# atsuki-ichikawa/KoeMorph

Measured on AMD Instinct MI355X. Metric: blendshape frames/sec (52-coef, 256-win, d_model=256), higher is better.
Workload: dtype f32; 1 GPU; C2: 256 windows/GPU x 136448 samples (8.5 s @16 kHz) -> 1024-pt STFT, hop 533, 80-bin log-mel (257 frames) -> dual-stream attention d_model=256, 8 heads, window 256 -> 52 coefficients + EMA; from audio resident in HBM (rotating batches); windows_per_gpu=256, samples_per_window=136448, parallelism=window-sharded x1, no collective

## Files before the change

include/koemorph.h:

```cpp
#ifndef KOEMORPH_H
#define KOEMORPH_H

#include <stdint.h>

#ifdef __cplusplus
extern "C" {
#endif

#define KM_ABI_VERSION 2

typedef enum km_status {
    KM_OK = 0,
    KM_ERR_INVALID_ARG = -1,
    KM_ERR_UNSUPPORTED = -2,
    KM_ERR_NOT_FINALIZED = -3,
    KM_ERR_WORKSPACE = -4,
    KM_ERR_HIP = -5,
    KM_ERR_NOT_READY = -6
} km_status;

typedef struct km_context* km_handle;

typedef enum km_mel_scale { KM_MEL_SLANEY = 0, KM_MEL_HTK = 1 } km_mel_scale;
typedef enum km_pad_mode { KM_PAD_CONSTANT = 0, KM_PAD_REFLECT = 1 } km_pad_mode;
// ... 121 lines not shown
    float ds_velocity_weight, ds_separation_weight;
    const float* ds_prev_pred_dev;
} km_loss_config;
int km_train_set_loss(km_handle h, const km_loss_config* cfg);
int km_audio_energy(const float* features_dev, int64_t B, int64_t T, int64_t D, float* energy_dev, void* stream);

int km_train_set_dropout(km_handle h, float p, uint64_t seed, int32_t external_masks);
int km_train_get_dropout_step(km_handle h, int64_t* step);
int km_train_set_dropout_step(km_handle h, int64_t step);

int km_train_grad_split(km_handle h, int64_t* early_floats);
int km_train_wait_early(km_handle h, void* stream);
int km_train_get_dropout_masks(km_handle h, int64_t B, uint8_t* mel_host, uint8_t* emo_host, uint8_t* dec_host, void* stream);
int km_train_set_dropout_masks(km_handle h, int64_t B, const uint8_t* mel_host, const uint8_t* emo_host, const uint8_t* dec_host,
                               void* stream);

typedef struct km_legacy_config {
    int32_t abi_version;
    int32_t d_model;
    int32_t num_heads;
    int32_t decoder_hidden;
    int32_t num_blendshapes;
    km_mel_config mel;
} km_legacy_config;
int km_legacy_create(const km_legacy_config* cfg, km_handle* out);
int km_legacy_forward(km_handle h, const float* audio_dev, int64_t B, int64_t L, float* out_dev, void* stream);
int km_legacy_forward_mel(km_handle h, const float* mel_dev, int64_t B, int64_t T_mel, float* out_dev, void* stream);

int km_legacy_train_init(km_handle h, int64_t max_windows, int64_t max_frames, void* stream);
int64_t km_legacy_train_num_params(km_handle h);
int64_t km_legacy_train_param_offset(km_handle h, const char* key);
int km_legacy_train_step_mel(km_handle h, const float* mel_dev, int64_t B, int64_t T, const float* target_dev, float mse_weight,
                             float l1_weight, float* flat_grad_dev, float* loss_dev, float* out_dev, void* stream);
int km_legacy_train_step_audio(km_handle h, const float* audio_dev, int64_t B, int64_t L, const float* target_dev, float mse_weight,
                               float l1_weight, float* flat_grad_dev, float* loss_dev, float* out_dev, void* stream);
int km_legacy_train_set_loss(km_handle h, const km_loss_config* cfg);
int km_legacy_train_adamw(km_handle h, const float* flat_grad_dev, float lr, float beta1, float beta2, float eps,
                          float weight_decay, float max_grad_norm, int64_t step, void* stream);
int km_legacy_train_get_params(km_handle h, float* flat_host, int64_t n);
int km_legacy_train_set_params(km_handle h, const float* flat_host, int64_t n);
int km_legacy_train_get_optimizer_state(km_handle h, float* exp_avg_host, float* exp_avg_sq_host, int64_t n, int32_t* steps2_host);
int km_legacy_train_set_optimizer_state(km_handle h, const float* exp_avg_host, const float* exp_avg_sq_host, int64_t n,
                                        const int32_t* steps2_host);
int km_legacy_train_sync(km_handle h, void* stream);
int km_legacy_train_set_dropout(km_handle h, float p, uint64_t seed, int32_t external_masks);
int km_legacy_train_get_dropout_step(km_handle h, int64_t* step);
int km_legacy_train_set_dropout_step(km_handle h, int64_t step);
int km_legacy_train_get_dropout_masks(km_handle h, int64_t B, int64_t T, uint8_t* enc1_host, uint8_t* enc2_host, uint8_t* attn_host,
                                      uint8_t* dec1_host, uint8_t* dec2_host, void* stream);
int km_legacy_train_set_dropout_masks(km_handle h, int64_t B, int64_t T, const uint8_t* enc1_host, const uint8_t* enc2_host,
                                      const uint8_t* attn_host, const uint8_t* dec1_host, const uint8_t* dec2_host, void* stream);

typedef struct km_koemorph_config {
    int32_t abi_version;
    int32_t mel_dim;
    int32_t emotion_dim;
    int32_t d_model;
    int32_t num_heads;
    int32_t num_encoder_layers;
    int32_t num_attention_layers;
    int32_t decoder_hidden_dim;
    int32_t decoder_layers;
    int32_t decoder_activation;
    int32_t causal;
    int32_t window_size;
    int32_t use_temporal_smoothing;
    int32_t use_constraints;
    int32_t num_blendshapes;
    int32_t output_activation;
    int32_t smoothing_method;
    int32_t smoothing_window;
} km_koemorph_config;
int km_koemorph_create(const km_koemorph_config* cfg, km_handle* out);
int km_koemorph_reserve(km_handle h, int64_t max_batch, int64_t max_frames);
int km_koemorph_forward(km_handle h, const float* mel_dev, const float* emotion_dev, int64_t B, int64_t T,
                        const uint8_t* audio_mask_dev, const float* prev_dev, float* smoother_state_dev,
                        int32_t apply_constraints, float* out_dev, float* raw_dev, float* attn_dev, void* stream);

int km_stream_create(km_handle h, int64_t n_streams, double context_window_s, double update_interval_s,
                     const km_mel_config* mel_cfg);
int km_stream_push(km_handle h, const float* samples_dev, int64_t n_per_stream, void* stream);
int km_stream_tick(km_handle h, const float* emotion_dev, float* out_dev, uint8_t* ready_dev, void* stream);
int km_stream_reset(km_handle h, void* stream);

int km_legacy_stream_create(km_handle h, int64_t n_streams, int64_t buffer_samples, int64_t audio_length);
int km_legacy_stream_push(km_handle h, const float* samples_dev, int64_t n_per_stream, const int32_t* counts_dev, void* stream);
int km_legacy_stream_tick(km_handle h, float* out_dev, uint8_t* ready_dev, void* stream);
int km_legacy_stream_reset(km_handle h, void* stream);

int km_enable_stage_timing(km_handle h, int32_t enable);
int km_stage_times(km_handle h, float* ms3);

int km_egemaps_plan_create(void** plan_out);
int km_egemaps_plan_destroy(void* plan);
int64_t km_egemaps_num_frames(int64_t L);
int64_t km_egemaps_workspace_floats(int64_t B, int64_t L);
int km_egemaps_functionals(void* plan, const float* audio_dev, int64_t B, int64_t L, int32_t normalize, float* work_dev,
                           int64_t work_floats, float* out_dev, void* stream);
int km_egemaps_records(const float* work_dev, int64_t B, int64_t L, float* rec_host, void* stream);
int km_egemaps_track_from_records(float* rec_dev, int64_t B, int64_t nf, void* stream);
int km_egemaps_functionals_from_records(const float* rec_dev, int64_t B, int64_t nf, float* out_dev, void* stream);
int km_linear(const float* x_dev, const float* w_dev, const float* b_dev, int64_t B, int64_t K, int64_t N, float* out_dev, void* stream);

#define KM_METRICS_COUNT 22
int km_metrics_create(void** acc_out);
int km_metrics_destroy(void* acc);
int km_metrics_reset(void* acc, void* stream);
int km_metrics_update(void* acc, const float* pred_dev, const float* target_dev, const float* audio_energy_dev, int64_t N, void* stream);
int km_metrics_compute(void* acc, float* out_dev, void* stream);

enum {
    KM_LOSS_TERM_MSE = 0, KM_LOSS_TERM_L1 = 1, KM_LOSS_TERM_PERCEPTUAL = 2, KM_LOSS_TERM_TEMPORAL = 3, KM_LOSS_TERM_VELOCITY = 4,
    KM_LOSS_TERM_SPARSITY = 5, KM_LOSS_TERM_SMOOTHNESS = 6, KM_LOSS_TERM_LANDMARK = 7, KM_LOSS_TERM_DS_VELOCITY = 8,
    KM_LOSS_TERM_DS_SEPARATION = 9, KM_LOSS_TERM_TOTAL = 10
};
#define KM_LOSS_TERMS 11
int km_loss_terms_create(void** acc_out);
int km_loss_terms_destroy(void* acc);
int km_loss_terms_reset(void* acc, void* stream);
int km_loss_terms_update(void* acc, const km_loss_config* cfg, float mse_weight, float l1_weight,
                         const float* pred_dev, const float* target_dev, int64_t N, float* terms_dev, void* stream);
int km_loss_terms_compute(void* acc, float* out_dev, void* stream);

int km_set_option(km_handle h, const char* name, int64_t value);

int km_debug_buffer(km_handle h, const char* name, float* out, int64_t* n);

int km_resample_labels(const float* src_dev, int64_t n_src, int32_t dims, int64_t n_dst, float* dst_dev, void* stream);
int km_gather_windows(const float* clip_dev, int64_t clip_len, const int32_t* start_frames_dev, int64_t B, int32_t hop,
                      int64_t window_samples, float* audio_out_dev, const float* labels_dev, int64_t n_label_frames,
                      int32_t window_frames, int32_t dims, float* labels_out_dev, float* target_out_dev, void* stream);

int64_t km_format_frames(const float* frames_host, int64_t n_frames, int32_t n_values, const double* timestamps,
                         int32_t newline, char* out, int64_t capacity, int64_t* offsets);

#ifdef __cplusplus
}
#endif
#endif
```

koemorph_amd/_lib.py:

```python
from __future__ import annotations

import ctypes as C
import os
from typing import Optional

from . import build as _build

KM_ABI_VERSION = 2


class KoeMorphError(RuntimeError):
    def __init__(self, code: int, msg: str):
        super().__init__(f"libkoemorph_hip: {msg} (status {code})")
        self.code = code


class KMMelConfig(C.Structure):
    _fields_ = [("sample_rate", C.c_int32), ("n_fft", C.c_int32), ("hop_length", C.c_int32),
                ("n_mels", C.c_int32), ("f_min", C.c_float), ("f_max", C.c_float),
                ("mel_scale", C.c_int32), ("slaney_norm", C.c_int32), ("pad_mode", C.c_int32),
                ("window_norm", C.c_int32), ("log_mode", C.c_int32), ("amin", C.c_float),
                ("top_db", C.c_float), ("db_add", C.c_float), ("db_scale", C.c_float),
                ("log_eps", C.c_float)]

# ... 47 lines not shown
_i64 = C.c_int64
_i32 = C.c_int32
_h = C.c_void_p

SIGNATURES = {
    "km_abi_version": (C.c_int, []),
    "km_last_error": (C.c_char_p, []),
    "km_create": (C.c_int, [C.POINTER(KMConfig), C.POINTER(_h)]),
    "km_destroy": (C.c_int, [_h]),
    "km_load_param": (C.c_int, [_h, C.c_char_p, _p, C.POINTER(_i64), _i32]),
    "km_get_param": (C.c_int, [_h, C.c_char_p, _p, _i64]),
    "km_param_count": (C.c_int, [_h, C.POINTER(_i32), C.POINTER(_i32)]),
    "km_finalize": (C.c_int, [_h, _p]),
    "km_finalize_host": (C.c_int, [_h]),
    "km_reserve": (C.c_int, [_h, _i64, _i64]),
    "km_mel_batch": (C.c_int, [_h, _p, _i64, _i64, _p, _p, _p]),
    "km_mel_num_frames": (_i64, [_h, _i64]),
    "km_mel_extract": (C.c_int, [_h, C.POINTER(KMMelConfig), _p, _i64, _i64, _i64, _p, _p]),
    "km_core_forward": (C.c_int, [_h, _p, _i64, _i64, _p, _p, _p, _p, _p, _p]),
    "km_emotion_logit": (C.c_int, [_h, _p, _i64, _p, _p]),
    "km_core_forward_z": (C.c_int, [_h, _p, _i64, _i64, _p, _p, _p, _p, _p, _p]),
    "km_smooth": (C.c_int, [_h, _p, _p, _i64, _i32, _p]),
    "km_forward_audio": (C.c_int, [_h, _p, _i64, _i64, _p, _p, _p, _i32, _p]),
    "km_forward_clip_supported": (C.c_int, [_h]),
    "km_forward_clip": (C.c_int, [_h, _p, _i64, _p, _i64, _i32, _i32, _p, _p, _p, _i32, _p]),
    "km_forward_audio_pipelined": (C.c_int, [_h, _p, _i64, _i64, _p, _p, _p, _i32, _p]),
    "km_pipeline_flush": (C.c_int, [_h, _p]),
    "km_sequence_num_outputs": (_i64, [_h, _i64, _i32]),
    "km_sequence_forward": (C.c_int, [_h, _p, _i64, _i64, _p, _i32, _i32, _p, _p]),
    "km_ema_scan": (C.c_int, [_h, _p, _i64, _i64, _p]),
    "km_train_init": (C.c_int, [_h, _i64, _p]),
    "km_train_num_params": (_i64, [_h]),
    "km_train_param_offset": (_i64, [_h, C.c_char_p]),
    "km_train_step": (C.c_int, [_h, _p, _i64, _i64, _p, _p, _p, C.c_float, C.c_float, _p, _p, _p, _p, _i32, _p]),
    "km_train_step_audio": (C.c_int, [_h, _p, _i64, _i64, _p, _p, C.c_float, C.c_float, _p, _p, _p, _p, _i32, _p]),
    "km_train_clip_supported": (C.c_int, [_h]),
    "km_train_step_clip": (C.c_int, [_h, _p, _i64, _p, _i64, _i32, _i32, _p, _p, C.c_float, C.c_float, _p, _p, _p, _p, _i32, _p]),
    "km_train_adamw": (C.c_int, [_h, _p, C.c_float, C.c_float, C.c_float, C.c_float, C.c_float, C.c_float, _i64, _p]),
    "km_train_get_params": (C.c_int, [_h, _p, _i64]),
    "km_train_set_params": (C.c_int, [_h, _p, _i64]),
    "km_train_sync": (C.c_int, [_h, _p]),
    "km_train_set_loss": (C.c_int, [_h, C.POINTER(KMLossConfig)]),
    "km_audio_energy": (C.c_int, [_p, _i64, _i64, _i64, _p, _p]),
    "km_train_set_dropout": (C.c_int, [_h, C.c_float, C.c_uint64, _i32]),
    "km_train_get_dropout_step": (C.c_int, [_h, C.POINTER(_i64)]),
    "km_train_set_dropout_step": (C.c_int, [_h, _i64]),
    "km_train_grad_split": (C.c_int, [_h, C.POINTER(_i64)]),
    "km_train_wait_early": (C.c_int, [_h, _p]),
    "km_train_get_dropout_masks": (C.c_int, [_h, _i64, _p, _p, _p, _p]),
    "km_train_set_dropout_masks": (C.c_int, [_h, _i64, _p, _p, _p, _p]),
    "km_train_get_optimizer_state": (C.c_int, [_h, _p, _p, _i64, _p]),
    "km_train_set_optimizer_state": (C.c_int, [_h, _p, _p, _i64, _p]),
    "km_resample_labels": (C.c_int, [_p, C.c_int64, C.c_int32, C.c_int64, _p, _p]),
    "km_gather_windows": (C.c_int, [_p, C.c_int64, _p, C.c_int64, C.c_int32, C.c_int64, _p, _p, C.c_int64, C.c_int32,
                                    C.c_int32, _p, _p, _p]),
    "km_format_frames": (C.c_int64, [_p, C.c_int64, C.c_int32, _p, C.c_int32, _p, C.c_int64, _p]),
    "km_legacy_create": (C.c_int, [C.POINTER(KMLegacyConfig), C.POINTER(_h)]),
    "km_legacy_forward": (C.c_int, [_h, _p, _i64, _i64, _p, _p]),
    "km_legacy_forward_mel": (C.c_int, [_h, _p, _i64, _i64, _p, _p]),
    "km_legacy_train_init": (C.c_int, [_h, _i64, _i64, _p]),
    "km_legacy_train_num_params": (_i64, [_h]),
    "km_legacy_train_param_offset": (_i64, [_h, C.c_char_p]),
    "km_legacy_train_step_mel": (C.c_int, [_h, _p, _i64, _i64, _p, C.c_float, C.c_float, _p, _p, _p, _p]),
    "km_legacy_train_step_audio": (C.c_int, [_h, _p, _i64, _i64, _p, C.c_float, C.c_float, _p, _p, _p, _p]),
    "km_legacy_train_set_loss": (C.c_int, [_h, C.POINTER(KMLossConfig)]),
    "km_legacy_train_adamw": (C.c_int, [_h, _p, C.c_float, C.c_float, C.c_float, C.c_float, C.c_float, C.c_float, _i64, _p]),
    "km_legacy_train_get_params": (C.c_int, [_h, _p, _i64]),
    "km_legacy_train_set_params": (C.c_int, [_h, _p, _i64]),
    "km_legacy_train_get_optimizer_state": (C.c_int, [_h, _p, _p, _i64, _p]),
    "km_legacy_train_set_optimizer_state": (C.c_int, [_h, _p, _p, _i64, _p]),
    "km_legacy_train_sync": (C.c_int, [_h, _p]),
    "km_legacy_train_set_dropout": (C.c_int, [_h, C.c_float, C.c_uint64, _i32]),
    "km_legacy_train_get_dropout_step": (C.c_int, [_h, C.POINTER(_i64)]),
    "km_legacy_train_set_dropout_step": (C.c_int, [_h, _i64]),
    "km_legacy_train_get_dropout_masks": (C.c_int, [_h, _i64, _i64, _p, _p, _p, _p, _p, _p]),
    "km_legacy_train_set_dropout_masks": (C.c_int, [_h, _i64, _i64, _p, _p, _p, _p, _p, _p]),
    "km_koemorph_create": (C.c_int, [C.POINTER(KMKoeMorphConfig), C.POINTER(_h)]),
    "km_koemorph_reserve": (C.c_int, [_h, _i64, _i64]),
    "km_koemorph_forward": (C.c_int, [_h, _p, _p, _i64, _i64, _p, _p, _p, _i32, _p, _p, _p, _p]),
    "km_stream_create": (C.c_int, [_h, _i64, C.c_double, C.c_double, C.POINTER(KMMelConfig)]),
    "km_stream_push": (C.c_int, [_h, _p, _i64, _p]),
    "km_stream_tick": (C.c_int, [_h, _p, _p, _p, _p]),
    "km_stream_reset": (C.c_int, [_h, _p]),
    "km_legacy_stream_create": (C.c_int, [_h, _i64, _i64, _i64]),
    "km_legacy_stream_push": (C.c_int, [_h, _p, _i64, _p, _p]),
    "km_legacy_stream_tick": (C.c_int, [_h, _p, _p, _p]),
    "km_legacy_stream_reset": (C.c_int, [_h, _p]),
    "km_set_option": (C.c_int, [_h, C.c_char_p, _i64]),
    "km_egemaps_plan_create": (C.c_int, [C.POINTER(_p)]),
    "km_egemaps_plan_destroy": (C.c_int, [_p]),
    "km_egemaps_num_frames": (_i64, [_i64]),
    "km_egemaps_workspace_floats": (_i64, [_i64, _i64]),
    "km_egemaps_functionals": (C.c_int, [_p, _p, _i64, _i64, _i32, _p, _i64, _p, _p]),
    "km_egemaps_records": (C.c_int, [_p, _i64, _i64, _p, _p]),
    "km_egemaps_track_from_records": (C.c_int, [_p, _i64, _i64, _p]),
    "km_egemaps_functionals_from_records": (C.c_int, [_p, _i64, _i64, _p, _p]),
    "km_metrics_create": (C.c_int, [C.POINTER(_p)]),
    "km_metrics_destroy": (C.c_int, [_p]),
    "km_metrics_reset": (C.c_int, [_p, _p]),
    "km_metrics_update": (C.c_int, [_p, _p, _p, _p, _i64, _p]),
    "km_metrics_compute": (C.c_int, [_p, _p, _p]),
    "km_loss_terms_create": (C.c_int, [C.POINTER(_p)]),
    "km_loss_terms_destroy": (C.c_int, [_p]),
    "km_loss_terms_reset": (C.c_int, [_p, _p]),
    "km_loss_terms_update": (C.c_int, [_p, C.POINTER(KMLossConfig), C.c_float, C.c_float, _p, _p, _i64, _p, _p]),
    "km_loss_terms_compute": (C.c_int, [_p, _p, _p]),
    "km_linear": (C.c_int, [_p, _p, _p, _i64, _i64, _i64, _p, _p]),
    "km_enable_stage_timing": (C.c_int, [_h, _i32]),
    "km_stage_times": (C.c_int, [_h, C.POINTER(C.c_float)]),
    "km_debug_buffer": (C.c_int, [_h, C.c_char_p, _p, C.POINTER(_i64)]),
}

_lib: Optional[C.CDLL] = None


def load(build_if_missing: bool = True) -> C.CDLL:
    global _lib
    if _lib is not None:
        return _lib
    path = _build.LIB_PATH
    if os.environ.get("KM_LIBRARY"):
        path, build_if_missing = os.environ["KM_LIBRARY"], False
    if build_if_missing and _build.is_stale():
        try:
            _build.build_library()
        except Exception as exc:
            if not os.path.exists(path) or os.environ.get("KM_ALLOW_STALE") != "1":
                raise KoeMorphError(KM_ERR_HIP, f"libkoemorph_hip.so is missing or older than its sources and the rebuild "
                                                f"failed ({exc}); set KM_ALLOW_STALE=1 to load the stale library") from exc
            import warnings
            warnings.warn(f"libkoemorph_hip.so is OLDER than its sources and the rebuild failed ({exc}); "
                          "loading the stale library (KM_ALLOW_STALE=1)", RuntimeWarning, stacklevel=2)
    if not os.path.exists(path):
        raise KoeMorphError(KM_ERR_HIP, f"{path} is missing: run `python -m koemorph_amd.build` "
                                        "(there is no CPU fallback)")
    import torch
    lib = C.CDLL(path)
    for name, (res, args) in SIGNATURES.items():
        fn = getattr(lib, name)
        fn.restype = res
        fn.argtypes = args
    if lib.km_abi_version() != KM_ABI_VERSION:
        raise KoeMorphError(KM_ERR_INVALID_ARG, "ABI version mismatch between _lib.py and the shared library")
    _lib = lib
    return lib


def check(code: int) -> None:
    if code != KM_OK:
        msg = load().km_last_error()
        raise KoeMorphError(code, msg.decode("utf-8", "replace") if msg else "unknown error")
```

koemorph_amd/csrc/km_api.hip:

```cpp
#include <hip/hip_runtime.h>

#include <cstdlib>

#include <cstring>
#include <vector>

#include "km_context.h"
#include "km_device.h"
#include "km_gemm.h"

using namespace km;

#define HIP_TRY(expr)                                                                         \
    do {                                                                                      \
        hipError_t e_ = (expr);                                                               \
        if (e_ != hipSuccess) {                                                                                                        \
            (void)hipGetLastError();  \
            return fail(KM_ERR_HIP, "%s: %s", #expr, hipGetErrorString(e_));                                                           \
        }                                                                                                                              \
    } while (0)

static int free_streams(Context* c);
static int free_train(Context* c);
static int free_pipeline(Context* c);
// ... 702 lines not shown
    c->kmm_batch = Bm; c->kmm_frames = Tm;
    return KM_OK;
}

int km_koemorph_forward(km_handle h, const float* mel_dev, const float* emotion_dev, int64_t B, int64_t T,
                        const uint8_t* audio_mask_dev, const float* prev_dev, float* smoother_state_dev,
                        int32_t apply_constraints, float* out_dev, float* raw_dev, float* attn_dev, void* stream) {
    if (int rc = need_ready(h)) return rc;
    Context* c = h;
    if (c->kind != 2) return fail(KM_ERR_INVALID_ARG, "not a KoeMorphModel handle (km_koemorph_create)");
    if (!mel_dev || !emotion_dev || !out_dev || B <= 0 || T <= 0) return fail(KM_ERR_INVALID_ARG, "km_koemorph_forward: bad argument");
    if (!c->ws_generic || B * koemorph_ws_floats(c, T) > c->kmm_batch * koemorph_ws_floats(c, c->kmm_frames))
        return fail(KM_ERR_WORKSPACE, "workspace too small for %lld x %lld frames: call km_koemorph_reserve", (long long)B, (long long)T);
    return launch_koemorph(c, mel_dev, emotion_dev, B, T, audio_mask_dev, prev_dev, smoother_state_dev, apply_constraints, out_dev, raw_dev,
                           attn_dev, stream);
}

int km_legacy_forward(km_handle h, const float* audio_dev, int64_t B, int64_t L, float* out_dev, void* stream) {
    if (int rc = need_ready(h)) return rc;
    Context* c = h;
    if (c->kind != 1) return fail(KM_ERR_INVALID_ARG, "not a legacy handle (km_legacy_create)");
    if (!audio_dev || !out_dev || B <= 0 || L <= 0) return fail(KM_ERR_INVALID_ARG, "km_legacy_forward: bad argument");
    const int64_t n_frames = 1 + L / c->cfg.mel.hop_length;
    if (B > c->ws_windows || n_frames > c->ws_frames || !c->ws_generic)
        return fail(KM_ERR_WORKSPACE, "workspace too small for %lld windows x %lld samples: call km_reserve",
                    (long long)B, (long long)L);
    if (legacy_pow_ok(c)) {
        if (int rc = launch_mel_power(c, c->mel_plans[0], mel_windows(audio_dev, B, L), stream)) return rc;
        const LogParams lp = plan_log_params(c->mel_plans[0]);
        const LegacyPowSrc src{c->ws_melpow, c->ws_melmax, &lp};
        return launch_legacy(c, nullptr, B, n_frames, out_dev, stream, &src);
    }
    if (int rc = launch_mel(c, c->mel_plans[0], mel_windows(audio_dev, B, L), 0, c->ws_mel, nullptr, stream)) return rc;
    return launch_legacy(c, c->ws_mel, B, n_frames, out_dev, stream);
}

int km_ema_scan(km_handle h, float* x_dev, int64_t B, int64_t N, void* stream) {
    if (int rc = need_ready(h)) return rc;
    if (h->kind != 0) return fail(KM_ERR_INVALID_ARG, "this entry point needs a dual-stream handle (km_create)");
    if (!x_dev || B <= 0 || N <= 0) return fail(KM_ERR_INVALID_ARG, "km_ema_scan: bad argument");
    return launch_ema_scan(h, x_dev, B, N, stream);
}

int km_smooth(km_handle h, float* x_dev, float* state_dev, int64_t B, int32_t first, void* stream) {
    if (int rc = need_ready(h)) return rc;
    if (!x_dev || !state_dev || B <= 0) return fail(KM_ERR_INVALID_ARG, "km_smooth: bad argument");
    return launch_smooth(h, x_dev, state_dev, B, first, stream);
}

int km_forward_audio(km_handle h, const float* audio_dev, int64_t B, int64_t L, const float* emotion_dev,
                     float* out_dev, float* state_dev, int32_t first, void* stream) {
    if (int rc = need_dual(h)) return rc;
    Context* c = h;
    if (!audio_dev || !emotion_dev || !out_dev || B <= 0 || L <= 0)
        return fail(KM_ERR_INVALID_ARG, "km_forward_audio: bad argument");
    const int64_t n_frames = 1 + L / c->cfg.mel.hop_length;
    if (B > c->ws_windows || n_frames > c->ws_frames)
        return fail(KM_ERR_WORKSPACE, "workspace too small for %lld windows x %lld samples: call km_reserve",
                    (long long)B, (long long)L);
    MelPlan* plan = c->mel_plans[0];
    const MelSrc src = mel_windows(audio_dev, B, L);
    if (!c->fused_ok) {
        if (!c->ws_generic) return fail(KM_ERR_WORKSPACE, "generic workspace missing: call km_reserve after km_finalize");
        const bool power_path = generic_core_takes_power(c) && !c->opt.generic_staged;
        const bool fuse_emo = power_path && mel_fuses_emotion(c, plan);
        if (!fuse_emo)
            if (int rc = launch_emotion(c, emotion_dev, B, c->ws_zemo, stream)) return rc;
        if (power_path) {
            if (int rc = launch_mel_power(c, plan, src, stream, fuse_emo ? mel_emotion(emotion_dev, c->ws_zemo) : MelCarry{})) return rc;
            if (int rc = launch_core_generic_power(c, plan, B, n_frames, c->ws_zemo, out_dev, nullptr, nullptr, stream)) return rc;
        } else if (c->NK == 80 && !c->opt.generic_staged) {
            float* xp = generic_packed_x(c, B);
            if (int rc = launch_mel_packed(c, plan, src, xp, c->T, (c->KT + 15) / 16 * 16, stream)) return rc;
            if (int rc = launch_core_generic_packed(c, xp, B, c->ws_zemo, out_dev, nullptr, nullptr, stream)) return rc;
        } else {
            if (int rc = launch_mel(c, plan, src, 0, c->ws_mel, c->ws_short, stream)) return rc;
            if (int rc = launch_core_generic(c, c->ws_mel, B, n_frames, c->ws_short, c->ws_zemo, out_dev, nullptr, nullptr, stream)) return rc;
        }
        if (state_dev) return launch_smooth(c, out_dev, state_dev, B, first, stream);
        return KM_OK;
    }
    hipStream_t st = (hipStream_t)stream;
    const bool tm = c->stage_timing;
    const bool fuse_emo = mel_fuses_emotion(c, plan);
    if (tm) HIP_TRY(hipEventRecord((hipEvent_t)c->stage_ev[0], st));
    if (!fuse_emo)
        if (int rc = launch_emotion(c, emotion_dev, B, c->ws_zemo, stream)) return rc;
    if (tm) HIP_TRY(hipEventRecord((hipEvent_t)c->stage_ev[1], st));
    if (int rc = launch_mel_power(c, plan, src, stream, fuse_emo ? mel_emotion(emotion_dev, c->ws_zemo) : MelCarry{})) return rc;
    if (tm) { HIP_TRY(hipEventRecord((hipEvent_t)c->stage_ev[2], st)); HIP_TRY(hipEventRecord((hipEvent_t)c->stage_ev[3], st)); }
    if (int rc = launch_core_fused_db(c, plan, B, n_frames, c->ws_zemo, out_dev, stream, core_workspace(state_dev, first))) return rc;
    if (tm) HIP_TRY(hipEventRecord((hipEvent_t)c->stage_ev[4], st));
    return KM_OK;
}

static bool forward_clip_ok(Context* c) {
    if (c->mel_plans.empty() || !c->fused_ok || c->opt.core_split == 3 || c->opt.core_split == 6) return false;
    return mel_rp_ok(c, c->mel_plans[0]) && clip_frames_shared(c, c->mel_plans[0]);
}

int km_forward_clip_supported(km_handle h) {
    if (!h || !h->dev_finalized || h->kind != 0) return 0;
    return forward_clip_ok(h) ? 1 : 0;
}

int km_forward_clip(km_handle h, const float* clip_dev, int64_t clip_len, const int32_t* start_frames_dev, int64_t B,
                    int32_t min_start_frame, int32_t max_start_frame, const float* emotion_dev, float* out_dev,
                    float* state_dev, int32_t first, void* stream) {
    if (int rc = need_dual(h)) return rc;
    Context* c = h;
    if (!clip_dev || !start_frames_dev || !emotion_dev || !out_dev || B <= 0 || clip_len <= 0 || min_start_frame < 0 ||
        max_start_frame < min_start_frame)
        return fail(KM_ERR_INVALID_ARG, "km_forward_clip: bad argument");
    const km_mel_config& m = c->mel_plans[0]->cfg;
    if (!forward_clip_ok(c))
        return fail(KM_ERR_UNSUPPORTED, "km_forward_clip: needs the fused core (d_model 256, window 256, 8 heads) behind the 1024-point "
                    "front end with constant padding and hop >= n_fft / 2 (hop %d, n_fft %d): gather the windows (km_gather_windows) "
                    "and call km_forward_audio", m.hop_length, m.n_fft);
    const int64_t T = c->T, hop = m.hop_length;
    const int64_t n_span = (int64_t)(max_start_frame - min_start_frame) + T + 1;
    if (clip_len >= (1ll << 31) || ((int64_t)max_start_frame + T + 2) * hop >= (1ll << 31) || n_span * c->NK >= (1ll << 31))
        return fail(KM_ERR_INVALID_ARG, "km_forward_clip: clip or start frame beyond 2^31 samples");
    if (B > c->ws_windows)
        return fail(KM_ERR_WORKSPACE, "workspace holds %lld windows, need %lld: call km_reserve", (long long)c->ws_windows, (long long)B);
    if (int rc = grow_buffer(&c->fwd_span, &c->fwd_span_cap, n_span, c->NK * sizeof(float), stream, "km_forward_clip: span frames")) return rc;
    if (int rc = grow_buffer(&c->fwd_edge, &c->fwd_edge_cap, B, 2 * c->NK * sizeof(float), stream, "km_forward_clip: windows")) return rc;
    if (int rc = launch_emotion(c, emotion_dev, B, c->ws_zemo, stream)) return rc;
    if (int rc = launch_mel_clip_span(c, c->mel_plans[0], clip_dev, clip_len, start_frames_dev, B, min_start_frame, n_span, (int)T,
                                      c->fwd_span, c->fwd_edge, stream)) return rc;
    if (int rc = launch_clip_window_max(c, c->fwd_span, c->fwd_edge, start_frames_dev, B, min_start_frame, n_span, (int)(T + 1),
                                        stream)) return rc;
    const ClipTable tab{c->fwd_span, c->fwd_edge, (int)n_span, start_frames_dev, min_start_frame};
    return launch_core_fused_db(c, c->mel_plans[0], B, T + 1, c->ws_zemo, out_dev, stream, core_table(&tab, state_dev, first));
}

static int free_streams(Context* c) {
    void* ptrs[] = {c->ring, c->ring_wptr, c->ring_frames, c->ring_ready, c->ring_started, c->ring_state};
    for (void* p : ptrs)
        if (p) HIP_TRY(hipFree(p));
    c->ring = nullptr; c->ring_wptr = nullptr; c->ring_frames = nullptr; c->ring_ready = nullptr;
    c->ring_started = nullptr; c->ring_state = nullptr; c->n_streams = 0;
    return KM_OK;
}

int km_stream_reset(km_handle h, void* stream) {
    if (int rc = need_dual(h)) return rc;
    Context* c = h;
    if (c->n_streams <= 0) return fail(KM_ERR_INVALID_ARG, "km_stream_reset: no streams (km_stream_create first)");
    hipStream_t st = (hipStream_t)stream;
    HIP_TRY(hipMemsetAsync(c->ring, 0, (size_t)c->n_streams * c->ring_len * sizeof(float), st));
    HIP_TRY(hipMemsetAsync(c->ring_wptr, 0, (size_t)c->n_streams * sizeof(int), st));
    HIP_TRY(hipMemsetAsync(c->ring_frames, 0, (size_t)c->n_streams * sizeof(int), st));
    HIP_TRY(hipMemsetAsync(c->ring_ready, 0, (size_t)c->n_streams, st));
    HIP_TRY(hipMemsetAsync(c->ring_started, 0, (size_t)c->n_streams, st));
    HIP_TRY(hipMemsetAsync(c->ring_state, 0, (size_t)c->n_streams * c->NB * sizeof(float), st));
    return KM_OK;
}

int km_stream_create(km_handle h, int64_t n_streams, double context_window_s, double update_interval_s,
                     const km_mel_config* mel_cfg) {
    if (int rc = need_dual(h)) return rc;
    Context* c = h;
    if (n_streams <= 0 || !(context_window_s > 0) || !(update_interval_s > 0) || !mel_cfg)
        return fail(KM_ERR_INVALID_ARG, "km_stream_create: bad argument");
    if (mel_cfg->n_fft != 512 && mel_cfg->n_fft != 1024) return fail(KM_ERR_UNSUPPORTED, "n_fft must be 512 or 1024");
    if (mel_cfg->n_mels != c->NK) return fail(KM_ERR_INVALID_ARG, "stream front end must produce %d mel channels", c->NK);
    if (int rc = free_streams(c)) return rc;
    const int sr = mel_cfg->sample_rate;
    c->ring_len = (int64_t)(context_window_s * sr);
    const double target_fps = 1.0 / update_interval_s;
    c->ring_hop = (int)((double)sr / target_fps);
    c->stream_out_frames = (int64_t)(context_window_s / update_interval_s);
    if (c->ring_hop <= 0 || c->ring_len <= mel_cfg->n_fft / 2) return fail(KM_ERR_INVALID_ARG, "context window too short");
    c->n_streams = n_streams;
    HIP_TRY(hipMalloc(reinterpret_cast<void**>(&c->ring), (size_t)n_streams * c->ring_len * sizeof(float)));
    HIP_TRY(hipMalloc(reinterpret_cast<void**>(&c->ring_wptr), (size_t)n_streams * sizeof(int)));
    HIP_TRY(hipMalloc(reinterpret_cast<void**>(&c->ring_frames), (size_t)n_streams * sizeof(int)));
    HIP_TRY(hipMalloc(reinterpret_cast<void**>(&c->ring_ready), (size_t)n_streams));
    HIP_TRY(hipMalloc(reinterpret_cast<void**>(&c->ring_started), (size_t)n_streams));
    HIP_TRY(hipMalloc(reinterpret_cast<void**>(&c->ring_state), (size_t)n_streams * c->NB * sizeof(float)));
    c->stream_plan = find_or_add_plan(c, *mel_cfg);
    if (int rc = upload_mel_plan(c->stream_plan)) return rc;
    if (int rc = km_reserve(h, n_streams, c->ring_len)) return rc;
    if (int rc = km_stream_reset(h, nullptr)) return rc;
    HIP_TRY(hipDeviceSynchronize());
    return KM_OK;
}

int km_stream_push(km_handle h, const float* samples_dev, int64_t n_per_stream, void* stream) {
    if (int rc = need_dual(h)) return rc;
    Context* c = h;
    if (c->n_streams <= 0) return fail(KM_ERR_INVALID_ARG, "km_stream_push: no streams (km_stream_create first)");
    if (!samples_dev) return fail(KM_ERR_INVALID_ARG, "km_stream_push: NULL samples");
    const int64_t diff = n_per_stream - c->ring_hop;
    if (diff > 1 || diff < -1)
        return fail(KM_ERR_INVALID_ARG, "Frame size mismatch: expected ~%d, got %lld", c->ring_hop, (long long)n_per_stream);
    return launch_ring_push(c, samples_dev, n_per_stream, stream);
}

int km_stream_tick(km_handle h, const float* emotion_dev, float* out_dev, uint8_t* ready_dev, void* stream) {
    if (int rc = need_dual(h)) return rc;
    Context* c = h;
    if (c->n_streams <= 0) return fail(KM_ERR_INVALID_ARG, "km_stream_tick: no streams (km_stream_create first)");
    if (!emotion_dev || !out_dev) return fail(KM_ERR_INVALID_ARG, "km_stream_tick: NULL argument");
    if (!c->fused_ok && !core512_stream_ok(c))
        return fail(KM_ERR_UNSUPPORTED, "no kernel for d_model=%d, mel_sequence_length=%d, heads=%d", c->d, c->T, c->H);
    const int64_t S = c->n_streams, L = c->ring_len;
    const int64_t n_frames = 1 + L / c->stream_plan->cfg.hop_length;
    if (S > c->ws_windows || n_frames > c->ws_frames) return fail(KM_ERR_WORKSPACE, "stream workspace too small");
    const bool fuse_emo = mel_fuses_emotion(c, c->stream_plan);
    if (!fuse_emo)
        if (int rc = launch_emotion(c, emotion_dev, S, c->ws_zemo, stream)) return rc;
    if (int rc = launch_mel_power(c, c->stream_plan, mel_rings(c), stream, fuse_emo ? mel_emotion(emotion_dev, c->ws_zemo) : MelCarry{})) return rc;
    if (c->fused_ok) {
        if (int rc = launch_core_fused_db(c, c->stream_plan, S, n_frames, c->ws_zemo, out_dev, stream, core_stream(c))) return rc;
    } else {
        if (int rc = launch_core512_stream(c, c->stream_plan, S, n_frames, c->ws_zemo, out_dev, stream)) return rc;
    }
    if (ready_dev)
        HIP_TRY(hipMemcpyAsync(ready_dev, c->ring_ready, (size_t)S, hipMemcpyDeviceToDevice, (hipStream_t)stream));
    return KM_OK;
}

static int free_legacy_streams(Context* c) {
    void* ptrs[] = {c->lfifo, c->lfifo_state, c->lfifo_stage, c->lfifo_ready, c->lfifo_attn};
    for (void* p : ptrs)
        if (p) HIP_TRY(hipFree(p));
    c->lfifo = nullptr; c->lfifo_state = nullptr; c->lfifo_stage = nullptr; c->lfifo_ready = nullptr; c->lfifo_attn = nullptr;
    c->lfifo_cap = c->lfifo_state_cap = c->lfifo_stage_cap = c->lfifo_ready_cap = c->lfifo_attn_cap = 0;
    c->lfifo_streams = c->lfifo_len = c->lfifo_window = 0;
    return KM_OK;
}

static bool legacy_stream_ok(Context* c) {
    return c->legacy_fused && c->legacy_tail_fused && c->d == 256 && c->H == 8 && c->legacy_hidden == 128 && c->NB == 52 && c->NK == 80 &&
           !c->mel_plans.empty() && c->mel_plans[0]->cfg.n_fft == 1024 && legacy_pow_ok(c);
}

static int need_legacy_stream(Context* c, const char* who) {
    if (int rc = need_ready(c)) return rc;
    if (c->kind != 1) return fail(KM_ERR_INVALID_ARG, "%s needs a legacy handle (km_legacy_create)", who);
    if (c->lfifo_streams <= 0) return fail(KM_ERR_INVALID_ARG, "%s: no streams (km_legacy_stream_create first)", who);
    return KM_OK;
}

int km_legacy_stream_reset(km_handle h, void* stream) {
    if (int rc = need_legacy_stream(h, "km_legacy_stream_reset")) return rc;
    Context* c = h;
    hipStream_t st = (hipStream_t)stream;
    const size_t S = (size_t)c->lfifo_streams;
    HIP_TRY(hipMemsetAsync(c->lfifo, 0, S * c->lfifo_len * sizeof(float), st));
    HIP_TRY(hipMemsetAsync(c->lfifo_stage, 0, S * c->lfifo_window * sizeof(float), st));
    HIP_TRY(hipMemsetAsync(c->lfifo_state, 0, 3 * S * sizeof(int), st));
    HIP_TRY(hipMemsetAsync(c->lfifo_ready, 0, S, st));
    return KM_OK;
}

int km_legacy_stream_create(km_handle h, int64_t n_streams, int64_t buffer_samples, int64_t audio_length) {
    if (int rc = need_ready(h)) return rc;
    Context* c = h;
    if (c->kind != 1) return fail(KM_ERR_INVALID_ARG, "km_legacy_stream_create needs a legacy handle (km_legacy_create)");
    if (n_streams <= 0 || buffer_samples <= 0 || audio_length <= 0 || audio_length > buffer_samples || n_streams >= (1ll << 24) ||
        buffer_samples >= (1ll << 30))
        return fail(KM_ERR_INVALID_ARG, "km_legacy_stream_create: bad argument (%lld streams, buffer of %lld samples, windows of %lld)",
                    (long long)n_streams, (long long)buffer_samples, (long long)audio_length);
    const int64_t T = 1 + audio_length / c->cfg.mel.hop_length;
    if (!legacy_stream_ok(c))
        return fail(KM_ERR_UNSUPPORTED, "km_legacy_stream_create: windows of %lld frames are served for d_model 256, 8 heads, decoder hidden 128 "
                    "behind the 1024-point front end only (got d_model %d, %d heads, hidden %d, n_fft %d)", (long long)T, c->d, c->H,
                    c->legacy_hidden, c->mel_plans.empty() ? 0 : c->mel_plans[0]->cfg.n_fft);
    if (T > 32)
        return fail(KM_ERR_UNSUPPORTED, "km_legacy_stream_create: windows of %lld samples are %lld frames, the stream kernel holds at most 32 "
                    "(use km_legacy_forward for longer windows)", (long long)audio_length, (long long)T);
    c->lfifo_streams = 0;
    const char* what = "km_legacy_stream_create";
    if (int rc = grow_buffer(&c->lfifo, &c->lfifo_cap, n_streams * buffer_samples, sizeof(float), nullptr, what)) return rc;
    if (int rc = grow_buffer(&c->lfifo_state, &c->lfifo_state_cap, 3 * n_streams, sizeof(int), nullptr, what)) return rc;
    if (int rc = grow_buffer(&c->lfifo_stage, &c->lfifo_stage_cap, n_streams * audio_length, sizeof(float), nullptr, what)) return rc;
    if (int rc = grow_buffer(&c->lfifo_ready, &c->lfifo_ready_cap, n_streams, 1, nullptr, what)) return rc;
    if (int rc = grow_buffer(&c->lfifo_attn, &c->lfifo_attn_cap, n_streams * c->NB * c->d, sizeof(float), nullptr, what)) return rc;
    if (int rc = km_reserve(h, n_streams, audio_length)) return rc;
    if (!legacy_stream_ok(c)) return fail(KM_ERR_UNSUPPORTED, "km_legacy_stream_create: the power-mel workspace is not 16-byte aligned");
    c->lfifo_streams = n_streams; c->lfifo_len = buffer_samples; c->lfifo_window = audio_length;
    HIP_TRY(hipMemset(c->ws_melmax, 0, (size_t)c->ws_windows * sizeof(unsigned)));
    c->melmax_dirty = false;
    if (int rc = km_legacy_stream_reset(h, nullptr)) return rc;
    if (int rc = km_legacy_stream_tick(h, c->lfifo_attn, nullptr, nullptr)) return rc;
    HIP_TRY(hipDeviceSynchronize());
    return KM_OK;
}

int km_legacy_stream_push(km_handle h, const float* samples_dev, int64_t n_per_stream, const int32_t* counts_dev, void* stream) {
    if (int rc = need_legacy_stream(h, "km_legacy_stream_push")) return rc;
    if (!samples_dev || n_per_stream <= 0 || n_per_stream >= (1ll << 30))
        return fail(KM_ERR_INVALID_ARG, "km_legacy_stream_push: bad argument");
    return launch_lfifo_push(h, samples_dev, n_per_stream, counts_dev, stream);
}

// ... 12 lines not shown

int km_enable_stage_timing(km_handle h, int32_t enable) {
    if (!h) return fail(KM_ERR_INVALID_ARG, "NULL handle");
    Context* c = h;
    if (enable && !c->stage_ev[0])
        for (int i = 0; i < 5; ++i) {
            hipEvent_t e;
            HIP_TRY(hipEventCreate(&e));
            c->stage_ev[i] = e;
        }
    c->stage_timing = enable != 0;
    return KM_OK;
}

int km_stage_times(km_handle h, float* ms3) {
    if (!h || !ms3) return fail(KM_ERR_INVALID_ARG, "km_stage_times: NULL argument");
    Context* c = h;
    if (!c->stage_ev[0]) return fail(KM_ERR_INVALID_ARG, "stage timing was never enabled");
    HIP_TRY(hipEventSynchronize((hipEvent_t)c->stage_ev[4]));
    HIP_TRY(hipEventElapsedTime(&ms3[0], (hipEvent_t)c->stage_ev[0], (hipEvent_t)c->stage_ev[1]));
    HIP_TRY(hipEventElapsedTime(&ms3[1], (hipEvent_t)c->stage_ev[1], (hipEvent_t)c->stage_ev[2]));
    HIP_TRY(hipEventElapsedTime(&ms3[2], (hipEvent_t)c->stage_ev[3], (hipEvent_t)c->stage_ev[4]));
    return KM_OK;
}

static int free_pipeline(Context* c) {
    for (int i = 0; i < 2; ++i) {
        if (c->pipe_melpow[i]) HIP_TRY(hipFree(c->pipe_melpow[i]));
        if (c->pipe_melmax[i]) HIP_TRY(hipFree(c->pipe_melmax[i]));
        if (c->pipe_zemo[i]) HIP_TRY(hipFree(c->pipe_zemo[i]));
        c->pipe_melpow[i] = nullptr; c->pipe_melmax[i] = nullptr; c->pipe_zemo[i] = nullptr; c->pipe_dirty[i] = true;
    }
    c->pipe_windows = c->pipe_frames = 0;
    return KM_OK;
}

static int ensure_pipeline(Context* c, int64_t B, int64_t n_frames) {
    if (!c->pipe_s1) {
        hipStream_t s;
        HIP_TRY(hipStreamCreateWithFlags(&s, hipStreamNonBlocking)); c->pipe_s1 = s;
        HIP_TRY(hipStreamCreateWithFlags(&s, hipStreamNonBlocking)); c->pipe_s2 = s;
        for (int i = 0; i < 2; ++i) {
            hipEvent_t e;
            HIP_TRY(hipEventCreateWithFlags(&e, hipEventDisableTiming)); c->pipe_ev_in[i] = e;
            HIP_TRY(hipEventCreateWithFlags(&e, hipEventDisableTiming)); c->pipe_ev_mel[i] = e;
            HIP_TRY(hipEventCreateWithFlags(&e, hipEventDisableTiming)); c->pipe_ev_core[i] = e;
        }
    }
    if (B <= c->pipe_windows && n_frames <= c->pipe_frames) return KM_OK;
    HIP_TRY(hipDeviceSynchronize());
    if (int rc = free_pipeline(c)) return rc;
    const int64_t W = B, F = n_frames;
    for (int i = 0; i < 2; ++i) {
        HIP_TRY(hipMalloc(reinterpret_cast<void**>(&c->pipe_melpow[i]), (size_t)W * F * c->NK * sizeof(float)));
        HIP_TRY(hipMalloc(reinterpret_cast<void**>(&c->pipe_melmax[i]), (size_t)W * sizeof(unsigned)));
        HIP_TRY(hipMalloc(reinterpret_cast<void**>(&c->pipe_zemo[i]), (size_t)W * sizeof(float)));
    }
    c->pipe_windows = W; c->pipe_frames = F; c->pipe_seq = 0;
    return KM_OK;
}

int km_forward_audio_pipelined(km_handle h, const float* audio_dev, int64_t B, int64_t L, const float* emotion_dev,
                               float* out_dev, float* state_dev, int32_t first, void* stream) {
    if (int rc = need_dual(h)) return rc;
    Context* c = h;
    if (!audio_dev || !emotion_dev || !out_dev || B <= 0 || L <= 0)
        return fail(KM_ERR_INVALID_ARG, "km_forward_audio_pipelined: bad argument");
    if (!c->fused_ok) return fail(KM_ERR_UNSUPPORTED, "the pipelined mode needs the fused kernel shape (d_model 256, window 256, 8 heads)");
    const int64_t n_frames = 1 + L / c->cfg.mel.hop_length;
    if (B > c->ws_windows || n_frames > c->ws_frames)
        return fail(KM_ERR_WORKSPACE, "workspace too small for %lld windows x %lld samples: call km_reserve", (long long)B, (long long)L);
    if (int rc = ensure_pipeline(c, B > c->ws_windows ? B : c->ws_windows, n_frames > c->ws_frames ? n_frames : c->ws_frames)) return rc;
    const int slot = (int)(c->pipe_seq & 1);
    hipStream_t caller = (hipStream_t)stream, s1 = (hipStream_t)c->pipe_s1, s2 = (hipStream_t)c->pipe_s2;
    const bool tm = c->stage_timing;
    float* keep_pow = c->ws_melpow; unsigned* keep_max = c->ws_melmax; float* keep_z = c->ws_zemo; const bool keep_dirty = c->melmax_dirty;
    c->ws_melpow = c->pipe_melpow[slot]; c->ws_melmax = c->pipe_melmax[slot]; c->ws_zemo = c->pipe_zemo[slot];
    c->melmax_dirty = c->pipe_dirty[slot];
    int rc = KM_OK;
    do {
        if (hipEventRecord((hipEvent_t)c->pipe_ev_in[slot], caller) != hipSuccess) { rc = fail(KM_ERR_HIP, "hipEventRecord failed"); break; }
        if (hipStreamWaitEvent(s1, (hipEvent_t)c->pipe_ev_in[slot], 0) != hipSuccess) { rc = fail(KM_ERR_HIP, "hipStreamWaitEvent failed"); break; }
        if (tm) (void)hipEventRecord((hipEvent_t)c->stage_ev[0], s1);
        const bool fuse_emo = mel_fuses_emotion(c, c->mel_plans[0]);
        if (!fuse_emo && (rc = launch_emotion(c, emotion_dev, B, c->ws_zemo, s1))) break;
        if (tm) (void)hipEventRecord((hipEvent_t)c->stage_ev[1], s1);
        if ((rc = launch_mel_power(c, c->mel_plans[0], mel_windows(audio_dev, B, L), s1, fuse_emo ? mel_emotion(emotion_dev, c->ws_zemo) : MelCarry{}))) break;
        if (tm) (void)hipEventRecord((hipEvent_t)c->stage_ev[2], s1);
        (void)hipEventRecord((hipEvent_t)c->pipe_ev_mel[slot], s1);
        (void)hipStreamWaitEvent(s2, (hipEvent_t)c->pipe_ev_mel[slot], 0);
        if (tm) (void)hipEventRecord((hipEvent_t)c->stage_ev[3], s2);
        if ((rc = launch_core_fused_db(c, c->mel_plans[0], B, n_frames, c->ws_zemo, out_dev, s2, core_workspace(state_dev, first)))) break;
        if (tm) (void)hipEventRecord((hipEvent_t)c->stage_ev[4], s2);
        (void)hipEventRecord((hipEvent_t)c->pipe_ev_core[slot], s2);
        if (c->pipe_seq > 0) (void)hipStreamWaitEvent(caller, (hipEvent_t)c->pipe_ev_core[slot ^ 1], 0);
    } while (0);
    c->pipe_dirty[slot] = c->melmax_dirty;
    c->ws_melpow = keep_pow; c->ws_melmax = keep_max; c->ws_zemo = keep_z; c->melmax_dirty = keep_dirty;
    if (rc == KM_OK) c->pipe_seq += 1;
    return rc;
}

int km_pipeline_flush(km_handle h, void* stream) {
    if (int rc = need_dual(h)) return rc;
    Context* c = h;
    if (c->pipe_seq > 0 && c->pipe_s1)
        HIP_TRY(hipStreamWaitEvent((hipStream_t)stream, (hipEvent_t)c->pipe_ev_core[(c->pipe_seq - 1) & 1], 0));
    return KM_OK;
}

int64_t km_sequence_num_outputs(km_handle h, int64_t L, int32_t stride_frames) {
    if (!h || L < 0 || stride_frames <= 0) return -1;
    const int64_t num_frames = L / h->cfg.mel.hop_length;
    const int64_t n = (num_frames - h->T) / stride_frames + 1;
    const int64_t nn = (num_frames - h->T) >= 0 ? n : ((num_frames - h->T - (stride_frames - 1)) / stride_frames + 1);
    return nn > 1 ? nn : 1;
}

int km_sequence_forward(km_handle h, const float* audio_dev, int64_t B, int64_t L, const float* emotion_dev,
                        int32_t stride_frames, int32_t smooth, float* out_dev, void* stream) {
    if (int rc = need_dual(h)) return rc;
    Context* c = h;
    if (!audio_dev || !emotion_dev || !out_dev || B <= 0 || L <= 0 || stride_frames <= 0)
        return fail(KM_ERR_INVALID_ARG, "km_sequence_forward: bad argument");
    if (!c->fused_ok && !c->ws_generic)
        return fail(KM_ERR_WORKSPACE, "generic workspace missing: call km_reserve after km_finalize");
    const int hop = c->cfg.mel.hop_length;
    const int64_t N = km_sequence_num_outputs(h, L, stride_frames);
    const int64_t W = (int64_t)c->T * hop;
    const int64_t step = (int64_t)stride_frames * hop;
    const int64_t n_frames = 1 + W / hop;
    if (c->ws_windows < B || c->ws_windows < 1 || n_frames > c->ws_frames)
        return fail(KM_ERR_WORKSPACE, "workspace too small for %lld clips / %lld-frame windows: call km_reserve",
                    (long long)B, (long long)n_frames);
    if (N > 0x7fffffff) return fail(KM_ERR_INVALID_ARG, "too many output frames");
    const int64_t total = B * N, tile = c->ws_windows;
    const bool dedup = !c->opt.seq_per_window;
    MelPlan* plan = c->mel_plans[0];
    const bool shared = c->fused_ok && dedup && mel_rp_ok(c, plan) && N < (1 << 24);
    const int64_t nfc = (N - 1) * stride_frames + n_frames;
    if (shared) {
        const char* what = "km_sequence_forward: clip frames / windows";
        if (int rc = grow_buffer(&c->seq_pow, &c->seq_pow_cap, B * nfc, c->NK * sizeof(float), stream, what)) return rc;
        if (int rc = grow_buffer(&c->seq_fmax, &c->seq_fmax_cap, B * nfc, sizeof(unsigned), stream, what)) return rc;
        if (int rc = grow_buffer(&c->seq_edge, &c->seq_edge_cap, total, 2 * c->NK * sizeof(float), stream, what)) return rc;
        if (int rc = grow_buffer(&c->seq_emax, &c->seq_emax_cap, total, 2 * sizeof(unsigned), stream, what)) return rc;
    }
    if (int rc = launch_emotion(c, emotion_dev, B, c->ws_zemo, stream)) return rc;
    if (shared) {
        hipStream_t st = (hipStream_t)stream;
        HIP_TRY(hipMemsetAsync(c->seq_fmax, 0, (size_t)B * nfc * sizeof(unsigned), st));
        HIP_TRY(hipMemsetAsync(c->seq_emax, 0, (size_t)total * 2 * sizeof(unsigned), st));
        const SeqFrames clip_img{c->seq_pow, c->seq_fmax, nfc, 1};
        if (int rc = launch_mel_power(c, plan, mel_clip_windows(audio_dev, L, B, (nfc - 1) * hop, 0, 0, 1), stream, mel_to_frames(&clip_img))) return rc;
        const SeqFrames edge_img{c->seq_edge, c->seq_emax, 2, (int)(n_frames - 1)};
        if (int rc = launch_mel_power(c, plan, mel_clip_windows(audio_dev, L, total, W, step, 0, (int)N), stream, mel_to_frames(&edge_img))) return rc;
        const SeqCore sc{c->seq_pow, c->seq_edge, (int)nfc, (int)stride_frames, (int)N};
        for (int64_t w0 = 0; w0 < total; w0 += tile) {
            const int64_t nw = (total - w0) < tile ? (total - w0) : tile;
            if (int rc = launch_seq_window_max(c, c->seq_fmax, c->seq_emax, nw, w0, (int)nfc, (int)stride_frames, (int)N,
                                               (int)n_frames, stream)) return rc;
            if (int rc = launch_core_fused_db(c, plan, nw, n_frames, c->ws_zemo, out_dev + w0 * c->NB, stream, core_strided(&sc, w0))) return rc;
        }
        if (smooth) return launch_ema_scan(c, out_dev, B, N, stream);
        return KM_OK;
    }
    for (int64_t w0 = 0; w0 < total; w0 += tile) {
        const int64_t nw = (total - w0) < tile ? (total - w0) : tile;
        const MelSrc src = mel_clip_windows(audio_dev, L, nw, W, step, w0, (int)N);
        if (c->fused_ok) {
            if (int rc = launch_mel_power(c, plan, src, stream)) return rc;
            if (int rc = launch_core_fused_db(c, plan, nw, n_frames, c->ws_zemo, out_dev + w0 * c->NB, stream, core_workspace_seq(w0, (int)N))) return rc;
        } else {
            if (int rc = launch_mel(c, plan, src, 0, c->ws_mel, c->ws_short, stream)) return rc;
            if (int rc = launch_gather_clip_logits(c, c->ws_zemo, c->ws_zemo_win, nw, w0, (int)N, stream)) return rc;
// ... 10 lines not shown
```

koemorph_amd/csrc/km_context.h:

```cpp
#pragma once

#include <cstdint>
#include <map>
#include <string>
#include <vector>

#include "koemorph.h"

namespace km {

constexpr int kNumMouth = 28;
constexpr int kNumExpr = 24;
extern const int kMouthIdx[kNumMouth];
extern const int kExprIdx[kNumExpr];

struct HostParam {
    std::vector<int64_t> shape;
    std::vector<float> data;
    bool loaded = false;
};

struct Packed {
    std::vector<float> host;
    float* dev = nullptr;
};

constexpr int kMelRpWaves = 8;
constexpr int kMelRpGroups = 4;
constexpr int kMelRpRow = 580;

struct MelPlan {
    km_mel_config cfg{};
    int n_freq = 0;
    std::vector<float> window;
    std::vector<float> twiddle;
    std::vector<int32_t> fb_start;
    std::vector<int32_t> fb_count;
    std::vector<int32_t> fb_offset;
    std::vector<float> fb_weight;
    std::vector<int32_t> fbg_gid;
    std::vector<int32_t> fbg_desc;
    std::vector<float> fbg_weight;
    int fbg_extent = 0;
    float* d_window = nullptr;
    float* d_twiddle = nullptr;
    int32_t* d_fb_start = nullptr;
    int32_t* d_fb_count = nullptr;
    int32_t* d_fb_offset = nullptr;
    float* d_fb_weight = nullptr;
    int32_t* d_fbg_gid = nullptr;
    int32_t* d_fbg_desc = nullptr;
    float* d_fbg_weight = nullptr;
    bool uploaded = false;
};

struct Options {
    int core_split = 0;
    int seq_per_window = 0;
    int generic_staged = 0;
    int mel_two_frame = 0;
    int emotion_separate = 0;
    int no_ln_fusion = 0, no_db_fusion = 0, no_score_fusion = 0, no_out_fusion = 0, no_v_fusion = 0;
    int legacy_no_merge = 0;
    int no_core_merge = 0;
    int legacy_no_tail_fusion = 0;
    int legacy_no_enc_fusion = 0;
    int legacy_no_attn_fusion = 0;
    int kmm_no_fuse = 0;
    int train_no_split = 0;
    int train_split_min_k = 0;
    int train_alone_max = 0;
    int train_no_dy_split = 0;
    int train_ln_fuse_rows = 0;
    int train_no_ln_fuse = 0;
    int train_colsum_gemm = 0;
    int train_no_fe_pack = 0;
    int train_attn_regs = 0;
    int train_no_dma = 0;
    int train_op_per_launch = 0;
    int train_bm32_below = 0;
    int train_tail_groups = 0;
};
void options_from_env(Options& o);
int set_option(struct Context* c, const char* name, long long value);

struct PerDeviceOnce {
    unsigned long long seen[4] = {0, 0, 0, 0};
    bool first(int device) {
        if (device < 0 || device >= 256) return true;
        const unsigned long long bit = 1ull << (device & 63);
        if (seen[device >> 6] & bit) return false;
        seen[device >> 6] |= bit;
        return true;
    }
};

struct Context {
    km_config cfg{};
    Options opt{};
    int kind = 0;
    int legacy_hidden = 128;
    km_koemorph_config kmm{};
    int64_t kmm_batch = 0, kmm_frames = 0;
    bool legacy_tail_fused = false;
    bool legacy_fused = false;
    bool kmm_fused = false;
    int d = 0, H = 0, hd = 0, T = 0, KT = 0, ED = 0, DH = 0, NB = 0, NK = 0;
    std::map<std::string, HostParam> params;
    std::vector<std::string> param_order;
    std::map<std::string, Packed> packed;
    bool host_finalized = false;
    bool dev_finalized = false;
    bool fused_ok = false;
    float alpha = 0.0f;
    int device = -1;

    std::vector<MelPlan*> mel_plans;

    int64_t ws_windows = 0, ws_samples = 0;
    float* ws_zemo = nullptr;
    float* ws_zemo_win = nullptr;
    float* ws_melpow = nullptr;
    unsigned* ws_melmax = nullptr;
    unsigned* ws_chunkctr = nullptr;
    int64_t ws_chunkctr_cap = 0;
    float* ws_mel = nullptr;
    float* ws_short = nullptr;
    float* ws_generic = nullptr;
    int64_t ws_frames = 0;
    int ws_mels = 0;
    int64_t n_streams = 0, ring_len = 0;
    int ring_hop = 0;
    float* ring = nullptr;
    int* ring_wptr = nullptr;
    int* ring_frames = nullptr;
    unsigned char* ring_ready = nullptr;
    unsigned char* ring_started = nullptr;
    float* ring_state = nullptr;
    MelPlan* stream_plan = nullptr;
    int64_t stream_out_frames = 0;
    int64_t lfifo_streams = 0, lfifo_len = 0, lfifo_window = 0;
    float* lfifo = nullptr; int64_t lfifo_cap = 0;
    int* lfifo_state = nullptr; int64_t lfifo_state_cap = 0;
    float* lfifo_stage = nullptr; int64_t lfifo_stage_cap = 0;
    unsigned char* lfifo_ready = nullptr; int64_t lfifo_ready_cap = 0;
    float* lfifo_attn = nullptr; int64_t lfifo_attn_cap = 0;
    int64_t tr_nparams = 0, tr_windows = 0;
    int64_t tr_early = 0;
    void* tr_early_ev = nullptr;
    bool tr_early_recorded = false;
    std::map<std::string, int64_t> tr_offset;
    float* tr_params = nullptr; float* tr_m = nullptr; float* tr_v = nullptr;
    float* trp_wcep = nullptr;
    float* tr_part = nullptr; float* tr_gnorm = nullptr; float* tr_loss = nullptr;
    int* tr_steps = nullptr;
    bool tr_alpha_live = false;
    km_loss_config tr_loss_cfg{};
    float* trp_act = nullptr; int64_t trp_act_floats = 0;
    float* trp_split = nullptr; int64_t trp_split_floats = 0;
    float* trp_tail_part = nullptr; unsigned* trp_tail_ctr = nullptr;
    void* trp_masks = nullptr;
    int* trp_drop_ctr = nullptr;
    float tr_dropout_p = 0.f;
    int tr_dropout_mode = 0;
    unsigned long long tr_dropout_seed = 0;
    float* ltr_ws = nullptr; int64_t ltr_ws_floats = 0;
    int64_t ltr_frames = 0;
    float* ltr_part = nullptr;
    unsigned char* ltr_masks = nullptr; int64_t ltr_mask_bytes = 0;
    int64_t ltr_mask_B = 0, ltr_mask_T = 0;
    float* seq_pow = nullptr; unsigned* seq_fmax = nullptr; float* seq_edge = nullptr; unsigned* seq_emax = nullptr;
    int64_t seq_pow_cap = 0, seq_fmax_cap = 0, seq_edge_cap = 0, seq_emax_cap = 0;
    float* fwd_span = nullptr; float* fwd_edge = nullptr;
    int64_t fwd_span_cap = 0, fwd_edge_cap = 0;
    float* clip_span = nullptr; float* clip_edge = nullptr;
    int64_t clip_span_cap = 0, clip_edge_cap = 0;
    int64_t tr_alpha_steps = 0;
    bool stage_timing = false;
    void* stage_ev[6] = {nullptr, nullptr, nullptr, nullptr, nullptr, nullptr};
    void* pipe_s1 = nullptr; void* pipe_s2 = nullptr;
    void* pipe_ev_in[2] = {nullptr, nullptr}; void* pipe_ev_mel[2] = {nullptr, nullptr}; void* pipe_ev_core[2] = {nullptr, nullptr};
    float* pipe_melpow[2] = {nullptr, nullptr}; unsigned* pipe_melmax[2] = {nullptr, nullptr}; float* pipe_zemo[2] = {nullptr, nullptr};
    bool pipe_dirty[2] = {true, true};
    int64_t pipe_seq = 0, pipe_windows = 0, pipe_frames = 0;
    bool melmax_dirty = true;
};

void set_error(const char* fmt, ...);
int fail(int code, const char* fmt, ...);

int finalize_host(Context* c);
MelPlan* build_mel_plan(const km_mel_config& cfg);
MelPlan* find_or_add_plan(Context* c, const km_mel_config& cfg);

int launch_emotion(Context* c, const float* emo, int64_t B, float* zemo, void* stream);
int launch_core_fused(Context* c, const float* mel, int64_t B, int64_t T_in, const float* mel_short,
                      const float* zemo, float* out, float* raw, float* attn, float* state, int first,
                      void* stream);
struct SeqCore {
    const float* pow;
    const float* edge;
    int nfc, stride, n_per_clip;
};
struct ClipTable {
    const float* span;
    const float* edge;
    int n_span;
    const int* start; int min_start;
};
struct CoreSrc {
    float* state; int first;
    int64_t win0; int zemo_div;
    int64_t n_use;
    const unsigned char* ready; unsigned char* started;
    const SeqCore* seq;
    const ClipTable* tab;
};
inline CoreSrc core_workspace(float* state, int first) { return {state, first, 0, 1, 0, nullptr, nullptr, nullptr, nullptr}; }
inline CoreSrc core_workspace_seq(int64_t win0, int n_per_clip) { return {nullptr, 1, win0, n_per_clip, 0, nullptr, nullptr, nullptr, nullptr}; }
inline CoreSrc core_strided(const SeqCore* s, int64_t win0) { return {nullptr, 1, win0, s->n_per_clip, 0, nullptr, nullptr, s, nullptr}; }
inline CoreSrc core_table(const ClipTable* t, float* state, int first) { return {state, first, 0, 1, 0, nullptr, nullptr, nullptr, t}; }
inline CoreSrc core_stream(Context* c) { return {c->ring_state, 0, 0, 1, c->stream_out_frames, c->ring_ready, c->ring_started, nullptr, nullptr}; }
int launch_core_fused_db(Context* c, MelPlan* p, int64_t B, int64_t n_frames, const float* zemo, float* out, void* stream,
                         const CoreSrc& src);
int launch_seq_window_max(Context* c, const unsigned* fmax, const unsigned* emax, int64_t nw, int64_t win0, int nfc, int stride,
                          int n_per_clip, int n_frames, void* stream);
int launch_clip_window_max(Context* c, const float* span, const float* edge, const int* start, int64_t B, int min_start,
                           int64_t n_span, int n_frames, void* stream);
int launch_ema_scan(Context* c, float* x, int64_t B, int64_t N, void* stream);
int launch_smooth(Context* c, float* x, float* state, int64_t B, int first, void* stream);

int train_refresh_padded_weights(Context* c, void* stream);
int train_adamw(Context* c, const float* flat_grad, float lr, float b1, float b2, float eps, float wd, float max_norm,
                int64_t step, void* stream);

int64_t trainp_act_floats(Context* c, int64_t* fixed);
int64_t trainp_kp(Context* c);
int64_t trainp_mask_alloc_bytes(Context* c);
int trainp_mask_sizes(Context* c, int64_t B, int64_t* mel, int64_t* emo, int64_t* dec);
int trainp_copy_masks(Context* c, int64_t B, unsigned char* mel, unsigned char* emo, unsigned char* dec, int to_device, void* stream);
struct LogParams;
struct TrainAudioSrc { const float* melpow; const unsigned* melmax; int n_frames; const LogParams* lp; bool packed; };
struct TrainStepArgs {
    const float* emo; const float* target; float mse_w, l1_w; float* flat_grad; float* loss_dev; float* out_dev;
    float* ema_state; int ema_first; void* stream;
};
int train_forward_backward(Context* c, const float* mel, int64_t B, int64_t T_in, const float* mel_short, const float* xp_dev,
                           const TrainAudioSrc* asrc, const TrainStepArgs& a);
int launch_audio_energy(const float* feats, int64_t B, int64_t T, int64_t D, float* out, void* stream);

bool legacy_train_supported(Context* c);
int legacy_train_init(Context* c, int64_t max_windows, int64_t max_frames, void* stream);
float* legacy_train_mel_buffer(Context* c);
int legacy_train_step(Context* c, const float* mel, int64_t B, int64_t T, const float* target, float mse_w, float l1_w, float* grad,
                      float* loss_dev, float* out_dev, void* stream);
int legacy_train_copy_masks(Context* c, int64_t B, int64_t T, unsigned char* const host[5], int to_device, void* stream);

int64_t generic_ws_floats(Context* c);
int64_t legacy_ws_floats(Context* c, int64_t frames);
int finalize_host_legacy(Context* c);
int finalize_host_koemorph(Context* c);
int64_t koemorph_ws_floats(Context* c, int64_t T);
int launch_koemorph(Context* c, const float* mel, const float* emo, int64_t B, int64_t T, const unsigned char* kvalid, const float* prev,
                    float* state, int apply_constraints, float* out, float* raw, float* attn, void* stream);
struct LegacyPowSrc { const float* melpow; unsigned* melmax; const LogParams* lp; };
bool legacy_pow_ok(Context* c);
int launch_legacy(Context* c, const float* mel, int64_t B, int64_t T_mel, float* out, void* stream, const LegacyPowSrc* pow_src = nullptr);
int launch_gather_clip_logits(Context* c, const float* zclip, float* zwin, int64_t nw, int64_t w0, int wins_per_clip, void* stream);
int launch_core_generic_packed(Context* c, const float* xp, int64_t B, const float* zemo, float* out, float* raw, float* attn,
                               void* stream);
float* generic_packed_x(Context* c, int64_t B);
bool generic_core_takes_power(Context* c);
int launch_core_generic_power(Context* c, MelPlan* plan, int64_t B, int64_t n_frames, const float* zemo, float* out,
                              float* raw, float* attn, void* stream);
int launch_core_generic(Context* c, const float* mel, int64_t B, int64_t T_in, const float* mel_short, const float* zemo,
                        float* out, float* raw, float* attn, void* stream);
bool core512_stream_ok(Context* c);
int launch_core512_stream(Context* c, MelPlan* plan, int64_t S, int64_t n_frames, const float* zemo, float* out, void* stream);

struct SeqFrames {
    float* pow;
    unsigned* fmax;
    int64_t n_rows;
    int frame_mul;
};
struct MelPack { float* xt; int T, KP; };
struct MelSrc {
    const float* audio; int64_t B, L;
    int64_t clip_len, win_step, win0; int wins_per_clip;
    const int* ring_start; const unsigned char* ready;
};
inline MelSrc mel_windows(const float* audio, int64_t B, int64_t L) { return {audio, B, L, L, 0, 0, 1, nullptr, nullptr}; }
inline MelSrc mel_clip_windows(const float* clips, int64_t clip_len, int64_t B, int64_t L, int64_t win_step, int64_t win0, int wins_per_clip) {
    return {clips, B, L, clip_len, win_step, win0, wins_per_clip, nullptr, nullptr};
}
inline MelSrc mel_rings(Context* c) { return {c->ring, c->n_streams, c->ring_len, c->ring_len, 0, 0, 1, c->ring_wptr, c->ring_ready}; }
struct MelCarry { const float* emotion = nullptr; float* zemo = nullptr; const SeqFrames* seq = nullptr; const MelPack* pack = nullptr; };
inline MelCarry mel_emotion(const float* emotion, float* zemo) { return {emotion, zemo, nullptr, nullptr}; }
inline MelCarry mel_to_frames(const SeqFrames* seq) { return {nullptr, nullptr, seq, nullptr}; }
inline MelCarry mel_to_pack(const MelPack* pack) { return {nullptr, nullptr, nullptr, pack}; }
int launch_mel_power(Context* c, MelPlan* p, const MelSrc& src, void* stream, const MelCarry& carry = {});
bool mel_rp_ok(Context* c, MelPlan* p);
bool clip_frames_shared(Context* c, MelPlan* p);
bool mel_packs(Context* c, MelPlan* p, int64_t n_frames, int64_t T);
int launch_mel_clip_span(Context* c, MelPlan* p, const float* clip, int64_t clip_len, const int* start_frames, int64_t B,
                         int min_start, int64_t n_span, int T, float* span, float* edge, void* stream);
int launch_train_clip_pack(Context* c, MelPlan* p, const float* span, const float* edge, const int* start_frames, int64_t B,
                           int min_start, int64_t n_span, int T, int KP, float* xt, void* stream);
bool mel_fuses_emotion(Context* c, MelPlan* p);
int ensure_chunk_counters(Context* c, int64_t windows, void* stream);
int growth_refused(void* stream, const char* what, int64_t need, int64_t cap);
int grow_buffer(void* ptr_addr, int64_t* cap, int64_t need, size_t unit_bytes, void* stream, const char* what);
int launch_ring_push(Context* c, const float* samples, int64_t n_per_stream, void* stream);

int launch_lfifo_push(Context* c, const float* samples, int64_t n_per_stream, const int* counts, void* stream);
int launch_lfifo_pop(Context* c, unsigned char* ready_out, void* stream);
int launch_legacy_stream_model(Context* c, const float* melpow, unsigned* melmax, const unsigned char* ready, int64_t S, int Tm,
                               const LogParams& lp, float* O, float* out, void* stream);
int launch_mel(Context* c, MelPlan* p, const MelSrc& src, int64_t out_frames, float* mel_long, float* mel_short, void* stream);
int launch_mel_packed(Context* c, MelPlan* p, const MelSrc& src, float* xp, int T, int KP, void* stream);
int upload_mel_plan(MelPlan* p);
void free_mel_plan(MelPlan* p);

}

struct km_context : public km::Context {};
```

koemorph_amd/csrc/km_core.hip:

```cpp
#include <hip/hip_runtime.h>

#include <type_traits>

#include "km_context.h"
#include "km_device.h"

namespace km {

typedef float f32x4 __attribute__((ext_vector_type(4)));
#define KM_MFMA(a, b, c) __builtin_amdgcn_mfma_f32_16x16x4f32((a), (b), (c), 0, 0, 0)

#define HIP_TRY(expr)                                                                         \
    do {                                                                                      \
        hipError_t e_ = (expr);                                                               \
        if (e_ != hipSuccess) {                                                                                                        \
            (void)hipGetLastError();  \
            return fail(KM_ERR_HIP, "%s: %s", #expr, hipGetErrorString(e_));                                                           \
        }                                                                                                                              \
    } while (0)

namespace fused {
constexpr int D = 256, T = 256, NK = 80, NQ = 28, DH = 128;
constexpr int KT = 259, KTP = 264, YS = 264, NW = 8, NT = 512;
constexpr int KP = 33;
constexpr int KB = 16;
constexpr int R1_FLOATS = KTP * NK;
constexpr int R2_FLOATS = 2 * NW * NK + 2 * NK;
constexpr int LDS_BYTES = (R1_FLOATS + R2_FLOATS) * 4;
constexpr int YSB = 264;
constexpr int PLANE_FLOATS = NK * YSB / 2;
constexpr int XSB = 296, XKB = 9;
constexpr int XPLANE_FLOATS = NK * XSB / 2;
constexpr int r1_floats(int np) { return np * XPLANE_FLOATS > R1_FLOATS ? np * XPLANE_FLOATS : R1_FLOATS; }
constexpr int lds_bytes(int np) { return (r1_floats(np) + R2_FLOATS) * 4; }
}

typedef __bf16 bf16x8 __attribute__((ext_vector_type(8)));
typedef unsigned int u32x4c __attribute__((ext_vector_type(4)));

struct CoreArgs {
    const float* mel;
    const float* mel_short;
    const float* zemo;
    int t_in;
    const float *wce_p, *bce, *ln_g, *ln_b, *qk_p, *wv_p, *wf_p, *bf, *w2, *b2, *wsum;
    const void* qkv_s;
    const void* wce_s;
    float* out;
    float* raw;
    float* attn;
    float* state;
    int first;
    float alpha;
    const float* melpow;
    unsigned* melmax;
    int n_frames;
    LogParams lp;
    int64_t win0;
    int zemo_div;
    int n_use;
    const float* seq_pow;
    const float* seq_edge;
    int seq_nfc, seq_stride, seq_n;
    const unsigned char* ready;
    unsigned char* started;
    const int* seq_start;
    int seq_min;
};

__device__ __forceinline__ int mouth_slot_of(int i) { return (i >= 14 && i <= 40) ? i - 14 : (i == 51 ? 27 : -1); }

template <bool ATTN, bool FUSE_DB, int NP = 0, bool TAB = false>
__global__ __launch_bounds__(512) void core_fused_kernel(CoreArgs a) {
    using namespace fused;
    extern __shared__ __attribute__((aligned(16))) float smem[];
    float* R1 = smem;
    float* R2 = smem + r1_floats(NP);

    const int b = blockIdx.x;
    const int tid = threadIdx.x;
    const int lane = tid & 63;
    const int wave = __builtin_amdgcn_readfirstlane(tid >> 6);
    const int g = lane >> 4, j = lane & 15;
    if constexpr (FUSE_DB) {
        if (a.ready && !a.ready[b]) return;
    }

    const int n0 = 32 * wave + j;
    float4 bw0 = make_float4(0.f, 0.f, 0.f, 0.f), bw1 = bw0;
    if constexpr (NP == 0) {
        const float4* wp0 = reinterpret_cast<const float4*>(a.wce_p) + (size_t)wave * KP * 64 + lane;
        bw0 = wp0[0];
    }
    const float bb0 = a.bce[n0], bb1 = a.bce[n0 + 16];
    const float g0 = a.ln_g[n0], g1 = a.ln_g[n0 + 16], be0 = a.ln_b[n0], be1 = a.ln_b[n0 + 16];
    float bf4[4], w24[4];
#pragma unroll
    for (int r = 0; r < 4; ++r) { bf4[r] = a.bf[16 * wave + 4 * g + r]; w24[r] = a.w2[16 * wave + 4 * g + r]; }
    const float tail_b2 = a.b2[0], tail_ws = tid < 52 ? a.wsum[tid] : 0.f;

    if constexpr (FUSE_DB) {
        float ref_db, floor_db;
        log_window_consts(a.lp, __uint_as_float(a.melmax[b]), ref_db, floor_db);
        const int F = a.n_frames;
        const int U = a.n_use;
        const int tv = U < T ? U : T;
        const float4* src = reinterpret_cast<const float4*>(a.melpow + (int64_t)b * F * NK);
        const float4 *seq_rows = nullptr, *seq_e = nullptr;
        if constexpr (TAB) {
            int r0 = a.seq_start[b];
            r0 = (r0 < 0 ? 0 : r0) - a.seq_min;
            r0 = r0 < 0 ? 0 : (r0 > a.seq_nfc - F ? a.seq_nfc - F : r0);
            seq_rows = reinterpret_cast<const float4*>(a.seq_pow + (int64_t)r0 * NK);
            seq_e = reinterpret_cast<const float4*>(a.seq_edge + (int64_t)b * 2 * NK);
        } else if (a.seq_pow) {
            const int64_t gw = a.win0 + b, clip = gw / a.seq_n, wi = gw - clip * a.seq_n;
            seq_rows = reinterpret_cast<const float4*>(a.seq_pow + (clip * a.seq_nfc + wi * a.seq_stride) * NK);
            seq_e = reinterpret_cast<const float4*>(a.seq_edge + gw * 2 * NK);
        }
        auto row4 = [&](int fr) -> const float4* {
            if (!seq_rows) return src + fr * 20;
            return fr == 0 ? seq_e : (fr == F - 1 ? seq_e + 20 : seq_rows + fr * 20);
        };
        float4* dst = reinterpret_cast<float4*>(R1);
        const float4 z4 = make_float4(0.f, 0.f, 0.f, 0.f);
        if constexpr (NP > 0) {
            auto src_row = [&](int t) -> int {
                if (t < T) return t < tv ? (t < F ? t : F - 1) : -1;
                if (t >= T + 3) return -1;
                const int r = t - T;
                int fr = -1;
                if (U >= 3) fr = U - 3 + r; else if (r < U) fr = r;
                return fr >= F ? F - 1 : fr;
            };
            auto stage_planes = [&](auto mode) {
                constexpr int MODE = decltype(mode)::value;
#pragma unroll 1
                for (int unit = tid; unit < XKB * 4 * 20; unit += NT) {
                    const int t8 = unit / 20, c4 = unit - t8 * 20;
                    float4 xv8[8];
                    unsigned okm = 0;
#pragma unroll
                    for (int q = 0; q < 8; ++q) {
                        const int fr = src_row(8 * t8 + q);
                        okm |= (fr >= 0 ? 1u : 0u) << q;
                        xv8[q] = fr >= 0 ? row4(fr)[c4] : z4;
                    }
                    float xe[4][8];
#pragma unroll
                    for (int q = 0; q < 8; ++q) {
                        const float4 v = (okm >> q) & 1 ? log_four_t<MODE>(a.lp, xv8[q], ref_db, floor_db) : z4;
                        xe[0][q] = v.x; xe[1][q] = v.y; xe[2][q] = v.z; xe[3][q] = v.w;
                    }
                    unsigned short* xp = reinterpret_cast<unsigned short*>(R1) + (4 * c4) * XSB + 8 * t8;
#pragma unroll
                    for (int pc = 0; pc < NP; ++pc)
#pragma unroll
                        for (int e = 0; e < 4; ++e) {
                            bf16x8 pk;
#pragma unroll
                            for (int q = 0; q < 8; ++q) {
                                const __bf16 pbf = (__bf16)xe[e][q];
                                pk[q] = pbf;
                                xe[e][q] -= (float)pbf;
                            }
                            *reinterpret_cast<bf16x8*>(xp + pc * (NK * XSB) + e * XSB) = pk;
                        }
                }
            };
            if (a.lp.log_mode == KM_LOG_LN_EPS) stage_planes(std::integral_constant<int, KM_LOG_LN_EPS>{});
            else stage_planes(std::integral_constant<int, KM_LOG_DB_MAX>{});
        } else {
        constexpr int NLD = T * 20 / NT;
        static_assert(NLD * NT == T * 20, "phase 0 assumes T*20 is a multiple of the workgroup size");
        float4 xv[NLD];
#pragma unroll
        for (int u = 0; u < NLD; ++u) {
            const int i = tid + NT * u;
            int fr = i / 20;
            const int c4 = i - fr * 20;
            fr = fr < F ? fr : F - 1;
            xv[u] = i < tv * 20 ? row4(fr)[c4] : z4;
        }
        float4 sv = z4;
        bool s_ok = false;
        if (tid < 60) {
            const int r = tid / 20;
            int fr = -1;
            if (U >= 3) fr = U - 3 + r; else if (r < U) fr = r;
            if (fr >= F) fr = F - 1;
            s_ok = fr >= 0;
            if (s_ok) sv = row4(fr)[tid - r * 20];
        }
        auto convert = [&](auto mode) {
            constexpr int MODE = decltype(mode)::value;
#pragma unroll
            for (int u = 0; u < NLD; ++u) {
                const int i = tid + NT * u;
                dst[i] = i < tv * 20 ? log_four_t<MODE>(a.lp, xv[u], ref_db, floor_db) : z4;
            }
            if (tid < 60) dst[T * 20 + tid] = s_ok ? log_four_t<MODE>(a.lp, sv, ref_db, floor_db) : z4;
        };
        if (a.lp.log_mode == KM_LOG_LN_EPS) convert(std::integral_constant<int, KM_LOG_LN_EPS>{});
        else convert(std::integral_constant<int, KM_LOG_DB_MAX>{});
        if (tid >= 64 && tid < 64 + (KTP - KT) * 20) dst[KT * 20 + tid - 64] = z4;
        }
    } else {
        const int tv = a.t_in < T ? a.t_in : T;
        const float4* src = reinterpret_cast<const float4*>(a.mel + (int64_t)b * a.t_in * NK);
        float4* dst = reinterpret_cast<float4*>(R1);
        const float4 z4 = make_float4(0.f, 0.f, 0.f, 0.f);
        for (int i = tid; i < tv * 20; i += NT) dst[i] = src[i];
        for (int i = tv * 20 + tid; i < T * 20; i += NT) dst[i] = z4;
        const float4* s4 = reinterpret_cast<const float4*>(a.mel_short + (int64_t)b * 3 * NK);
        if (tid < 60) dst[T * 20 + tid] = s4[tid];
        if (tid >= 64 && tid < 64 + (KTP - KT) * 20) dst[KT * 20 + tid - 64] = z4;
    }
    __syncthreads();
    if constexpr (FUSE_DB) {
        if (tid == 0) a.melmax[b] = 0u;
    }

    f32x4 acc[5][2];
#pragma unroll
    for (int mt = 0; mt < 5; ++mt) { acc[mt][0] = f32x4{0, 0, 0, 0}; acc[mt][1] = f32x4{0, 0, 0, 0}; }
    if constexpr (NP > 0) {
        const u32x4c* wp = reinterpret_cast<const u32x4c*>(a.wce_s) + (size_t)wave * XKB * 2 * NP * 64 + lane;
        const unsigned short* Xp = reinterpret_cast<const unsigned short*>(R1) + j * XSB + 8 * g;
        u32x4c bw[2][NP];
#pragma unroll
        for (int t = 0; t < 2; ++t)
#pragma unroll
            for (int pc = 0; pc < NP; ++pc) bw[t][pc] = wp[(t * NP + pc) * 64];
        for (int kb = 0; kb < XKB; ++kb) {
            const int kn = kb + 1 < XKB ? kb + 1 : kb;
            u32x4c bn[2][NP];
#pragma unroll
            for (int t = 0; t < 2; ++t)
#pragma unroll
                for (int pc = 0; pc < NP; ++pc) bn[t][pc] = wp[((kn * 2 + t) * NP + pc) * 64];
#pragma unroll
            for (int mt = 0; mt < 5; ++mt) {
                bf16x8 ap[NP];
#pragma unroll
                for (int pc = 0; pc < NP; ++pc)
                    ap[pc] = __builtin_bit_cast(bf16x8, *reinterpret_cast<const u32x4c*>(Xp + pc * (NK * XSB) + 16 * mt * XSB + 32 * kb));
#pragma unroll
                for (int t = 0; t < 2; ++t) {
                    f32x4 c4 = acc[mt][t];
                    if constexpr (NP == 3) {
                        c4 = __builtin_amdgcn_mfma_f32_16x16x32_bf16(ap[1], __builtin_bit_cast(bf16x8, bw[t][1]), c4, 0, 0, 0);
                        c4 = __builtin_amdgcn_mfma_f32_16x16x32_bf16(ap[0], __builtin_bit_cast(bf16x8, bw[t][2]), c4, 0, 0, 0);
                        c4 = __builtin_amdgcn_mfma_f32_16x16x32_bf16(ap[2], __builtin_bit_cast(bf16x8, bw[t][0]), c4, 0, 0, 0);
                    }
                    c4 = __builtin_amdgcn_mfma_f32_16x16x32_bf16(ap[0], __builtin_bit_cast(bf16x8, bw[t][1]), c4, 0, 0, 0);
                    c4 = __builtin_amdgcn_mfma_f32_16x16x32_bf16(ap[1], __builtin_bit_cast(bf16x8, bw[t][0]), c4, 0, 0, 0);
                    c4 = __builtin_amdgcn_mfma_f32_16x16x32_bf16(ap[0], __builtin_bit_cast(bf16x8, bw[t][0]), c4, 0, 0, 0);
                    acc[mt][t] = c4;
                }
            }
#pragma unroll
            for (int t = 0; t < 2; ++t)
#pragma unroll
                for (int pc = 0; pc < NP; ++pc) bw[t][pc] = bn[t][pc];
        }
    } else {
        const float4* wp = reinterpret_cast<const float4*>(a.wce_p) + (size_t)wave * KP * 64 + lane;
        float4 bw = bw0;
        for (int kp = 0; kp < KP; ++kp) {
            const float4 bn = wp[(size_t)(kp + 1 < KP ? kp + 1 : kp) * 64];
#pragma unroll
            for (int ds = 0; ds < 2; ++ds) {
                const float* xr = R1 + (4 * (2 * kp + ds) + g) * NK + j;
                const float b0 = ds ? bw.z : bw.x, b1 = ds ? bw.w : bw.y;
                float av[5];
#pragma unroll
                for (int mt = 0; mt < 5; ++mt) av[mt] = xr[16 * mt];
#pragma unroll
                for (int mt = 0; mt < 5; ++mt) {
                    acc[mt][0] = KM_MFMA(av[mt], b0, acc[mt][0]);
                    acc[mt][1] = KM_MFMA(av[mt], b1, acc[mt][1]);
                }
            }
            bw = bn;
        }
    }
    f32x4 q0 = f32x4{0, 0, 0, 0}, q1 = q0, v0 = q0, v1 = q0;
    if constexpr (NP == 0) {
        const f32x4* qp0 = reinterpret_cast<const f32x4*>(a.qk_p) + (size_t)wave * KB * 2 * 64 + lane;
        const f32x4* vp0 = reinterpret_cast<const f32x4*>(a.wv_p) + (size_t)wave * KB * 2 * 64 + lane;
        q0 = qp0[0]; q1 = qp0[64]; v0 = vp0[0]; v1 = vp0[64];
    }
    {
#pragma unroll
        for (int mt = 0; mt < 5; ++mt)
#pragma unroll
            for (int r = 0; r < 4; ++r) { acc[mt][0][r] += bb0; acc[mt][1][r] += bb1; }
    }
    float mean[5][4], rstd[5][4];
#pragma unroll
    for (int pass = 0; pass < 2; ++pass) {
        float part[5][4];
#pragma unroll
        for (int mt = 0; mt < 5; ++mt)
#pragma unroll
            for (int r = 0; r < 4; ++r) {
                float v;
                if (pass == 0) {
                    v = acc[mt][0][r] + acc[mt][1][r];
                } else {
                    const float d0 = acc[mt][0][r] - mean[mt][r], d1 = acc[mt][1][r] - mean[mt][r];
                    v = d0 * d0 + d1 * d1;
                }
                part[mt][r] = row16_sum(v);
            }
        float* P = R2 + pass * (NW * NK);
        if (j == 0) {
#pragma unroll
            for (int mt = 0; mt < 5; ++mt)
#pragma unroll
                for (int r = 0; r < 4; ++r) P[(16 * mt + 4 * g + r) * NW + wave] = part[mt][r];
        }
        __syncthreads();
        float* Tt = R2 + 2 * NW * NK + pass * NK;
        if (lane < NK / NW) {
            const int row = wave * (NK / NW) + lane;
            const f32x4* pr = reinterpret_cast<const f32x4*>(P + row * NW);
            const f32x4 lo = pr[0], hi = pr[1];
            float s = 0.f;
            s += lo[0]; s += lo[1]; s += lo[2]; s += lo[3];
            s += hi[0]; s += hi[1]; s += hi[2]; s += hi[3];
            Tt[row] = s;
        }
        __syncthreads();
#pragma unroll
        for (int mt = 0; mt < 5; ++mt) {
            const f32x4 t4 = *reinterpret_cast<const f32x4*>(Tt + 16 * mt + 4 * g);
#pragma unroll
            for (int r = 0; r < 4; ++r) {
                if (pass == 0) mean[mt][r] = t4[r] * (1.0f / D);
                else rstd[mt][r] = __builtin_amdgcn_rsqf(t4[r] * (1.0f / D) + 1e-5f);
            }
        }
    }
    {
#pragma unroll
        for (int mt = 0; mt < 5; ++mt)
#pragma unroll
            for (int r = 0; r < 4; ++r) {
                const float y0 = (acc[mt][0][r] - mean[mt][r]) * rstd[mt][r] * g0 + be0;
                const float y1 = (acc[mt][1][r] - mean[mt][r]) * rstd[mt][r] * g1 + be1;
                if constexpr (NP == 0) {
                    float* yr = R1 + (16 * mt + 4 * g + r) * YS + n0;
                    yr[0] = y0;
                    yr[16] = y1;
                } else {
                    unsigned short* yp = reinterpret_cast<unsigned short*>(R1) + (16 * mt + 4 * g + r) * YSB + n0;
                    float r0 = y0, r1 = y1;
#pragma unroll
                    for (int pc = 0; pc < NP; ++pc) {
                        const __bf16 p0 = (__bf16)r0, p1 = (__bf16)r1;
                        yp[pc * (NK * YSB)] = __builtin_bit_cast(unsigned short, p0);
                        yp[pc * (NK * YSB) + 16] = __builtin_bit_cast(unsigned short, p1);
                        r0 -= (float)p0;
                        r1 -= (float)p1;
                    }
                }
            }
    }
    __syncthreads();

    f32x4 S[5][2], V[5][2];
#pragma unroll
    for (int mt = 0; mt < 5; ++mt) {
        S[mt][0] = f32x4{0, 0, 0, 0}; S[mt][1] = f32x4{0, 0, 0, 0};
        V[mt][0] = f32x4{0, 0, 0, 0}; V[mt][1] = f32x4{0, 0, 0, 0};
    }
    if constexpr (NP > 0) {
        const u32x4c* wp = reinterpret_cast<const u32x4c*>(a.qkv_s) + (size_t)wave * 8 * 4 * NP * 64 + lane;
        const unsigned short* Yp = reinterpret_cast<const unsigned short*>(R1) + j * YSB + 8 * g;
        u32x4c bw[4][NP];
#pragma unroll
        for (int t = 0; t < 4; ++t)
#pragma unroll
            for (int pc = 0; pc < NP; ++pc) bw[t][pc] = wp[(t * NP + pc) * 64];
        for (int kb = 0; kb < 8; ++kb) {
            const int kn = kb + 1 < 8 ? kb + 1 : kb;
            u32x4c bn[4][NP];
#pragma unroll
            for (int t = 0; t < 4; ++t)
#pragma unroll
                for (int pc = 0; pc < NP; ++pc) bn[t][pc] = wp[((kn * 4 + t) * NP + pc) * 64];
#pragma unroll
            for (int mt = 0; mt < 5; ++mt) {
                bf16x8 ap[NP];
#pragma unroll
                for (int pc = 0; pc < NP; ++pc)
                    ap[pc] = __builtin_bit_cast(bf16x8, *reinterpret_cast<const u32x4c*>(Yp + pc * (NK * YSB) + 16 * mt * YSB + 32 * kb));
#pragma unroll
                for (int t = 0; t < 4; ++t) {
                    f32x4 c4 = t < 2 ? S[mt][t] : V[mt][t - 2];
                    if constexpr (NP == 3) {
                        c4 = __builtin_amdgcn_mfma_f32_16x16x32_bf16(ap[1], __builtin_bit_cast(bf16x8, bw[t][1]), c4, 0, 0, 0);
                        c4 = __builtin_amdgcn_mfma_f32_16x16x32_bf16(ap[0], __builtin_bit_cast(bf16x8, bw[t][2]), c4, 0, 0, 0);
                        c4 = __builtin_amdgcn_mfma_f32_16x16x32_bf16(ap[2], __builtin_bit_cast(bf16x8, bw[t][0]), c4, 0, 0, 0);
                    }
                    c4 = __builtin_amdgcn_mfma_f32_16x16x32_bf16(ap[0], __builtin_bit_cast(bf16x8, bw[t][1]), c4, 0, 0, 0);
                    c4 = __builtin_amdgcn_mfma_f32_16x16x32_bf16(ap[1], __builtin_bit_cast(bf16x8, bw[t][0]), c4, 0, 0, 0);
                    c4 = __builtin_amdgcn_mfma_f32_16x16x32_bf16(ap[0], __builtin_bit_cast(bf16x8, bw[t][0]), c4, 0, 0, 0);
                    if (t < 2) S[mt][t] = c4; else V[mt][t - 2] = c4;
                }
            }
#pragma unroll
            for (int t = 0; t < 4; ++t)
#pragma unroll
                for (int pc = 0; pc < NP; ++pc) bw[t][pc] = bn[t][pc];
        }
// ... 54 lines not shown
#pragma unroll
    for (int mt = 0; mt < 5; ++mt)
#pragma unroll
        for (int r = 0; r < 4; ++r) {
            O[0][0] = KM_MFMA(V[mt][0][r], S[mt][0][r], O[0][0]);
            O[0][1] = KM_MFMA(V[mt][0][r], S[mt][1][r], O[0][1]);
            O[1][0] = KM_MFMA(V[mt][1][r], S[mt][0][r], O[1][0]);
            O[1][1] = KM_MFMA(V[mt][1][r], S[mt][1][r], O[1][1]);
        }

    __syncthreads();
#pragma unroll
    for (int dt = 0; dt < 2; ++dt)
#pragma unroll
        for (int qt = 0; qt < 2; ++qt)
            *reinterpret_cast<f32x4*>(R1 + (16 * qt + j) * YS + 32 * wave + 16 * dt + 4 * g) = O[dt][qt];

    if constexpr (ATTN) {
        float* Pa = R1 + 32 * YS;
        for (int h = 0; h < NW; ++h) {
            if (wave == h) {
#pragma unroll
                for (int qt = 0; qt < 2; ++qt) {
                    const int q = 16 * qt + j;
                    if (q < NQ) {
#pragma unroll
                        for (int mt = 0; mt < 5; ++mt)
#pragma unroll
                            for (int r = 0; r < 4; ++r) {
                                float* p = Pa + q * NK + 16 * mt + 4 * g + r;
                                *p = (h == 0 ? 0.f : *p) + S[mt][qt][r];
                            }
                    }
                }
            }
            __syncthreads();
        }
        float* ao = a.attn + (int64_t)b * NQ * NK;
        for (int i = tid; i < NQ * NK; i += NT) ao[i] = Pa[i] * (1.0f / NW);
    } else {
        __syncthreads();
    }

    f32x4 Z[2];
    Z[0] = f32x4{0, 0, 0, 0}; Z[1] = f32x4{0, 0, 0, 0};
    {
        const f32x4* fp = reinterpret_cast<const f32x4*>(a.wf_p) + (size_t)wave * KB * 64 + lane;
#pragma unroll 4
        for (int kb = 0; kb < KB; ++kb) {
            const f32x4 wa = fp[(size_t)kb * 64];
            const f32x4 o0 = *reinterpret_cast<const f32x4*>(R1 + j * YS + 16 * kb + 4 * g);
            const f32x4 o1 = *reinterpret_cast<const f32x4*>(R1 + (16 + j) * YS + 16 * kb + 4 * g);
#pragma unroll
            for (int s = 0; s < 4; ++s) {
                Z[0] = KM_MFMA(wa[s], o0[s], Z[0]);
                Z[1] = KM_MFMA(wa[s], o1[s], Z[1]);
            }
        }
    }
    {
        float zp[2] = {0.f, 0.f};
#pragma unroll
        for (int r = 0; r < 4; ++r) {
            const float bfv = bf4[r], w2v = w24[r];
            zp[0] += fmaxf(Z[0][r] + bfv, 0.f) * w2v;
            zp[1] += fmaxf(Z[1][r] + bfv, 0.f) * w2v;
        }
#pragma unroll
        for (int qt = 0; qt < 2; ++qt) {
            zp[qt] += __shfl_xor(zp[qt], 16);
            zp[qt] += __shfl_xor(zp[qt], 32);
        }
        if (g == 0) { R2[wave * 32 + j] = zp[0]; R2[wave * 32 + 16 + j] = zp[1]; }
    }
    __syncthreads();
    if (tid < 52) {
        const int slot = mouth_slot_of(tid);
        float z;
        if (slot >= 0) {
            z = tail_b2;
#pragma unroll
            for (int w = 0; w < NW; ++w) z += R2[w * 32 + slot];
        } else {
            z = a.zemo[(a.win0 + b) / a.zemo_div];
        }
        const float bs = 1.0f / (1.0f + expf(-z));
        float val = fminf(fmaxf(tail_ws * bs, 0.f), 1.f);
        if (a.raw) a.raw[(int64_t)b * 52 + tid] = bs;
        if (a.state) {
            float* st = a.state + (int64_t)b * 52 + tid;
            const bool first = a.started ? !a.started[b] : (a.first != 0);
            if (!first) val = a.alpha * val + (1.0f - a.alpha) * (*st);
            *st = val;
        }
        a.out[(int64_t)b * 52 + tid] = val;
    }
    if constexpr (FUSE_DB) {
        __syncthreads();
        if (tid == 0 && a.started) a.started[b] = 1;
    }
}

constexpr int EWPB = 4;
constexpr int ENT = 1024;
constexpr int EKQ1 = 4;
constexpr int EKQ2 = 8;

__global__ __launch_bounds__(1024) void emotion_kernel(const float* __restrict__ emo, int64_t B, int ED, int d, int DH,
                                                       const float* __restrict__ wee_t, const float* __restrict__ bee,
                                                       const float* __restrict__ lg, const float* __restrict__ lb,
                                                       const float* __restrict__ we2, const float* __restrict__ be2,
                                                       const float* __restrict__ w2, const float* __restrict__ b2,
                                                       float* __restrict__ zemo) {
    extern __shared__ __attribute__((aligned(16))) float es[];
    float* emo_s = es;
    float* e1 = emo_s + EWPB * ED;
    float* part = e1 + EWPB * d;
    const int tid = threadIdx.x, lane = tid & 63, wave = tid >> 6;
    const int64_t b0 = (int64_t)blockIdx.x * EWPB;
    const int nb = (int)((B - b0) < EWPB ? (B - b0) : EWPB);
    for (int i = tid; i < EWPB * ED; i += ENT) {
        const int w = i / ED;
        emo_s[i] = w < nb ? emo[b0 * ED + i] : 0.f;
    }
    __syncthreads();
    {
        const int kq = tid >> 8, kchunk = (ED + EKQ1 - 1) / EKQ1;
        const int k0 = kq * kchunk, k1 = (k0 + kchunk) < ED ? (k0 + kchunk) : ED;
        for (int n = tid & 255; n < d; n += 256) {
            float acc[EWPB];
#pragma unroll
            for (int w = 0; w < EWPB; ++w) acc[w] = 0.f;
            const float* wp = wee_t + n;
            int k = k0;
            for (; k + 16 <= k1; k += 16) {
                float wv[16];
#pragma unroll
                for (int u = 0; u < 16; ++u) wv[u] = wp[(size_t)(k + u) * d];
#pragma unroll
                for (int u = 0; u < 16; ++u)
#pragma unroll
                    for (int w = 0; w < EWPB; ++w) acc[w] = fmaf(emo_s[w * ED + k + u], wv[u], acc[w]);
            }
            for (; k < k1; ++k) {
                const float wv = wp[(size_t)k * d];
#pragma unroll
                for (int w = 0; w < EWPB; ++w) acc[w] = fmaf(emo_s[w * ED + k], wv, acc[w]);
            }
#pragma unroll
            for (int w = 0; w < EWPB; ++w) part[(kq * EWPB + w) * d + n] = acc[w];
        }
    }
    __syncthreads();
    for (int i = tid; i < EWPB * d; i += ENT) {
        const int w = i / d, n = i - w * d;
        float s = bee[n];
#pragma unroll
        for (int kq = 0; kq < EKQ1; ++kq) s += part[(kq * EWPB + w) * d + n];
        e1[i] = s;
    }
    __syncthreads();
    if (wave < EWPB) {
        const int w = wave;
        float s = 0.f;
        for (int n = lane; n < d; n += 64) s += e1[w * d + n];
#pragma unroll
        for (int o = 32; o > 0; o >>= 1) s += __shfl_xor(s, o);
// ... 210 lines not shown
    a.qk_p = dv(c, "qk_p"); a.wv_p = dv(c, "wv_p"); a.wf_p = dv(c, "wf_p"); a.bf = dv(c, "bf");
    a.w2 = dv(c, "w2"); a.b2 = dv(c, "b2"); a.wsum = dv(c, "wsum");
    a.alpha = c->alpha;
}

int launch_core_fused(Context* c, const float* mel, int64_t B, int64_t T_in, const float* mel_short,
                      const float* zemo, float* out, float* raw, float* attn, float* state, int first,
                      void* stream) {
    if (int rc = core_attrs(c)) return rc;
    CoreArgs a{};
    core_weights(c, a);
    a.mel = mel; a.mel_short = mel_short; a.zemo = zemo; a.t_in = (int)T_in;
    a.out = out; a.raw = raw; a.attn = attn; a.state = state; a.first = first; a.win0 = 0; a.zemo_div = 1;
    if (attn)
        hipLaunchKernelGGL((core_fused_kernel<true, false>), dim3((unsigned)B), dim3(fused::NT), fused::LDS_BYTES, (hipStream_t)stream, a);
    else
        hipLaunchKernelGGL((core_fused_kernel<false, false>), dim3((unsigned)B), dim3(fused::NT), fused::LDS_BYTES, (hipStream_t)stream, a);
    HIP_TRY(hipGetLastError());
    return KM_OK;
}

LogParams plan_log_params(MelPlan* p);

__global__ __launch_bounds__(64) void seq_window_max_kernel(const unsigned* __restrict__ fmax, const unsigned* __restrict__ emax,
                                                            unsigned* __restrict__ melmax, int64_t win0, int nfc, int stride,
                                                            int n_per_clip, int n_frames) {
    const int64_t gw = win0 + blockIdx.x, clip = gw / n_per_clip, wi = gw - clip * n_per_clip;
    const unsigned* f = fmax + clip * nfc + wi * stride;
    unsigned m = 0;
    for (int r = 1 + threadIdx.x; r < n_frames - 1; r += 64) m = max(m, f[r]);
    if (threadIdx.x < 2) m = max(m, emax[gw * 2 + threadIdx.x]);
#pragma unroll
    for (int o = 32; o > 0; o >>= 1) m = max(m, (unsigned)__shfl_xor((int)m, o));
    if (threadIdx.x == 0) melmax[blockIdx.x] = m;
}

int launch_seq_window_max(Context* c, const unsigned* fmax, const unsigned* emax, int64_t nw, int64_t win0, int nfc, int stride,
                          int n_per_clip, int n_frames, void* stream) {
    hipLaunchKernelGGL(seq_window_max_kernel, dim3((unsigned)nw), dim3(64), 0, (hipStream_t)stream, fmax, emax, c->ws_melmax,
                       win0, nfc, stride, n_per_clip, n_frames);
    HIP_TRY(hipGetLastError());
    c->melmax_dirty = false;
    return KM_OK;
}

constexpr int CWM_NT = 256;
__global__ __launch_bounds__(CWM_NT) void clip_window_max_kernel(const float* __restrict__ span, const float* __restrict__ edge,
                                                                 const int* __restrict__ start, unsigned* __restrict__ melmax,
                                                                 int min_start, int n_span, int n_frames, int nk4) {
    __shared__ float red[CWM_NT / 64];
    const int b = blockIdx.x, tid = threadIdx.x;
    int r0 = start[b];
    r0 = (r0 < 0 ? 0 : r0) - min_start;
    r0 = r0 < 0 ? 0 : (r0 > n_span - n_frames ? n_span - n_frames : r0);
    const float4* rows = reinterpret_cast<const float4*>(span) + (int64_t)(r0 + 1) * nk4;
    const float4* e = reinterpret_cast<const float4*>(edge) + (int64_t)b * 2 * nk4;
    float m = 0.f;
    auto take = [&](const float4 v) { m = fmaxf(m, fmaxf(fmaxf(v.x, v.y), fmaxf(v.z, v.w))); };
    const int n_in = (n_frames - 2) * nk4;
    for (int i = tid; i < n_in; i += CWM_NT) take(rows[i]);
    for (int i = tid; i < 2 * nk4; i += CWM_NT) take(e[i]);
#pragma unroll
    for (int o = 32; o > 0; o >>= 1) m = fmaxf(m, __shfl_xor(m, o));
    if ((tid & 63) == 0) red[tid >> 6] = m;
    __syncthreads();
    if (tid == 0) {
        float mx = red[0];
#pragma unroll
        for (int w = 1; w < CWM_NT / 64; ++w) mx = fmaxf(mx, red[w]);
        melmax[b] = __float_as_uint(mx);
    }
}

int launch_clip_window_max(Context* c, const float* span, const float* edge, const int* start, int64_t B, int min_start,
                           int64_t n_span, int n_frames, void* stream) {
    if (!span || !edge || !start || B <= 0 || n_frames < 3 || n_span < n_frames || c->NK % 4 != 0)
        return fail(KM_ERR_INVALID_ARG, "clip window maximum: bad argument");
    hipLaunchKernelGGL(clip_window_max_kernel, dim3((unsigned)B), dim3(CWM_NT), 0, (hipStream_t)stream, span, edge, start, c->ws_melmax,
                       min_start, (int)n_span, n_frames, c->NK / 4);
    HIP_TRY(hipGetLastError());
    return KM_OK;
}

int launch_core_fused_db(Context* c, MelPlan* p, int64_t B, int64_t n_frames, const float* zemo, float* out, void* stream,
                         const CoreSrc& src) {
    if (int rc = core_attrs(c)) return rc;
    CoreArgs a{};
    core_weights(c, a);
    a.zemo = zemo; a.t_in = (int)n_frames;
    a.out = out; a.state = src.state; a.first = src.first; a.win0 = src.win0; a.zemo_div = src.zemo_div > 0 ? src.zemo_div : 1;
    a.melpow = c->ws_melpow; a.melmax = c->ws_melmax; a.n_frames = (int)n_frames; a.lp = plan_log_params(p);
    a.n_use = (int)(src.n_use > 0 ? src.n_use : n_frames); a.ready = src.ready; a.started = src.started;
    if (const SeqCore* s = src.seq) { a.seq_pow = s->pow; a.seq_edge = s->edge; a.seq_nfc = s->nfc; a.seq_stride = s->stride; a.seq_n = s->n_per_clip; }
    if (const ClipTable* t = src.tab) {
        if (src.seq || c->opt.core_split == 3 || c->opt.core_split == 6)
            return fail(KM_ERR_UNSUPPORTED, "fused core: a start-frame table goes with neither strided images nor the split-bf16 variant");
        a.seq_pow = t->span; a.seq_edge = t->edge; a.seq_nfc = t->n_span; a.seq_stride = 0; a.seq_n = 1;
        a.seq_start = t->start; a.seq_min = t->min_start;
        hipLaunchKernelGGL((core_fused_kernel<false, true, 0, true>), dim3((unsigned)B), dim3(fused::NT), fused::LDS_BYTES, (hipStream_t)stream, a);
        HIP_TRY(hipGetLastError());
        return KM_OK;
    }
    const int terms = c->opt.core_split;
    if (terms == 3) {
        a.qkv_s = dv(c, "qkv_s2"); a.wce_s = dv(c, "wce_s2");
        hipLaunchKernelGGL((core_fused_kernel<false, true, 2>), dim3((unsigned)B), dim3(fused::NT), fused::lds_bytes(2), (hipStream_t)stream, a);
    } else if (terms == 6) {
        a.qkv_s = dv(c, "qkv_s3"); a.wce_s = dv(c, "wce_s3");
        hipLaunchKernelGGL((core_fused_kernel<false, true, 3>), dim3((unsigned)B), dim3(fused::NT), fused::lds_bytes(3), (hipStream_t)stream, a);
    } else {
        hipLaunchKernelGGL((core_fused_kernel<false, true>), dim3((unsigned)B), dim3(fused::NT), fused::LDS_BYTES, (hipStream_t)stream, a);
    }
    HIP_TRY(hipGetLastError());
    return KM_OK;
}

__global__ void ema_scan_kernel(float* __restrict__ x, int64_t B, int64_t N, int nb, float alpha) {
    const int64_t i = (int64_t)blockIdx.x * blockDim.x + threadIdx.x;
    if (i >= B * nb) return;
    const int64_t b = i / nb;
    const int cidx = (int)(i - b * nb);
    float* p = x + b * N * nb + cidx;
    float prev = p[0];
    for (int64_t t = 1; t < N; ++t) {
        const float v = alpha * p[t * nb] + (1.0f - alpha) * prev;
        p[t * nb] = v;
        prev = v;
    }
}

int launch_ema_scan(Context* c, float* x, int64_t B, int64_t N, void* stream) {
    const int64_t n = B * c->NB;
    hipLaunchKernelGGL(ema_scan_kernel, dim3((unsigned)((n + 127) / 128)), dim3(128), 0, (hipStream_t)stream, x, B, N,
                       c->NB, c->alpha);
    HIP_TRY(hipGetLastError());
    return KM_OK;
}

int launch_smooth(Context* c, float* x, float* state, int64_t B, int first, void* stream) {
    const int64_t n = B * c->NB;
    hipLaunchKernelGGL(smooth_kernel, dim3((unsigned)((n + 255) / 256)), dim3(256), 0, (hipStream_t)stream, x, state, n,
                       first, c->alpha);
    HIP_TRY(hipGetLastError());
    return KM_OK;
}

}
```

koemorph_amd/csrc/km_device.h:

```cpp
#pragma once

#include <hip/hip_runtime.h>

#include "koemorph.h"

namespace km {

struct LogParams {
    int log_mode;
    float amin, top_db, db_add, db_scale, log_eps;
};

__device__ __forceinline__ float clamp_lo(float x, float lo) { return __builtin_amdgcn_fmed3f(x, lo, __builtin_inff()); }
__device__ __forceinline__ float db10(float s, float amin) {
    return 3.01029995663981195f * __builtin_amdgcn_logf(clamp_lo(s, amin));
}

__device__ __forceinline__ void log_window_consts(const LogParams& p, float ref, float& ref_db, float& floor_db) {
    ref_db = db10(ref, p.amin);
    floor_db = (db10(ref, p.amin) - ref_db) - p.top_db;
}

__device__ __forceinline__ float db_finish(const LogParams& p, float dbs, float ref_db, float floor_db) {
    float v = dbs - ref_db;
    v = clamp_lo(v, floor_db);
    return (v + p.db_add) * p.db_scale;
}
__device__ __forceinline__ float db_fast_c1(const LogParams& p, float ref_db) { return (p.db_add - ref_db) * p.db_scale; }
__device__ __forceinline__ float db_finish_fast(float dbs, float scale, float c1) { return fmaxf(fmaf(dbs, scale, c1), 0.f); }
struct DbXform { LogParams lp; const unsigned* ref_bits; };

struct LnXform { const float* stats; const float* gamma; const float* beta; int npart; float eps; };
__device__ __forceinline__ void ln_combine(const float2* __restrict__ st, int npart, float eps, float& rs, float& nmurs, float* mean_out = nullptr) {
    float msum = 0.f;
    for (int p = 0; p < npart; ++p) msum += st[p].x;
    const float mean = msum / (float)npart;
    float m2 = 0.f;
    for (int p = 0; p < npart; ++p) { const float dm = st[p].x - mean; m2 += st[p].y + 32.0f * dm * dm; }
    rs = 1.0f / sqrtf(m2 / (float)(32 * npart) + eps);
    nmurs = -mean * rs;
    if (mean_out) *mean_out = mean;
}
__device__ __forceinline__ void ln_combine8(const float2 (&st)[8], int npart, float eps, float& rs, float& nmurs) {
    float msum = 0.f;
#pragma unroll
    for (int p = 0; p < 8; ++p) msum += p < npart ? st[p].x : 0.f;
    const float mean = msum / (float)npart;
    float m2 = 0.f;
#pragma unroll
    for (int p = 0; p < 8; ++p) { const float dm = st[p].x - mean; m2 += p < npart ? st[p].y + 32.0f * dm * dm : 0.f; }
    rs = 1.0f / sqrtf(m2 / (float)(32 * npart) + eps);
    nmurs = -mean * rs;
}
__device__ __forceinline__ float ln_apply(float x, float rs, float nmurs, float gam, float bet) { return fmaf(fmaf(x, rs, nmurs), gam, bet); }

template <int MODE>
__device__ __forceinline__ float log_one_t(const LogParams& p, float s, float ref_db, float floor_db) {
    if (MODE == KM_LOG_LN_EPS) return 0.693147180559945309f * __builtin_amdgcn_logf(s + p.log_eps);
    float v = db10(s, p.amin) - ref_db;
    v = clamp_lo(v, floor_db);
    return (v + p.db_add) * p.db_scale;
}

__device__ __forceinline__ float log_one(const LogParams& p, float s, float ref_db, float floor_db) {
    return p.log_mode == KM_LOG_LN_EPS ? log_one_t<KM_LOG_LN_EPS>(p, s, ref_db, floor_db)
                                       : log_one_t<KM_LOG_DB_MAX>(p, s, ref_db, floor_db);
}

template <int MODE>
__device__ __forceinline__ float4 log_four_t(const LogParams& p, float4 v, float ref_db, float floor_db) {
    return make_float4(log_one_t<MODE>(p, v.x, ref_db, floor_db), log_one_t<MODE>(p, v.y, ref_db, floor_db),
                       log_one_t<MODE>(p, v.z, ref_db, floor_db), log_one_t<MODE>(p, v.w, ref_db, floor_db));
}

__device__ __forceinline__ float row16_sum(float v) {
    v += __int_as_float(__builtin_amdgcn_update_dpp(0, __float_as_int(v), 0xB1, 0xF, 0xF, true));
    v += __int_as_float(__builtin_amdgcn_update_dpp(0, __float_as_int(v), 0x4E, 0xF, 0xF, true));
    v += __int_as_float(__builtin_amdgcn_update_dpp(0, __float_as_int(v), 0x141, 0xF, 0xF, true));
    v += __int_as_float(__builtin_amdgcn_update_dpp(0, __float_as_int(v), 0x140, 0xF, 0xF, true));
    return v;
}

struct EmoArgs {
    const float* emo = nullptr;
    int ED = 0;
    const float *wee_t = nullptr , *bee = nullptr, *lg = nullptr, *lb = nullptr, *we2 = nullptr, *be2 = nullptr,
                *w2 = nullptr, *b2 = nullptr;
    float* zemo = nullptr;
    int d = 256, DH = 128;
};

__device__ __forceinline__ void emotion_window_d256(const EmoArgs& e, int64_t b, float* scratch) {
    constexpr int d = 256, DH = 128;
    float* emo_s = scratch;
    float* e1 = scratch + 256;
    float* part = scratch + 512;
    const int tid = threadIdx.x, lane = tid & 63;
    if (tid < 256) emo_s[tid] = tid < e.ED ? e.emo[b * e.ED + tid] : 0.f;
    __syncthreads();
    {
        const int n = tid & 255, h = __builtin_amdgcn_readfirstlane(tid >> 8);
#pragma unroll 1
        for (int q = 2 * h; q < 2 * h + 2; ++q) {
            const float* wp = e.wee_t + (size_t)64 * q * d + n;
            float w[64];
#pragma unroll
            for (int u = 0; u < 64; ++u) w[u] = wp[u * d];
            float acc = 0.f;
#pragma unroll
            for (int u = 0; u < 64; u += 4) {
                const float4 x = *reinterpret_cast<const float4*>(emo_s + 64 * q + u);
                acc = fmaf(x.x, w[u], acc);
                acc = fmaf(x.y, w[u + 1], acc);
                acc = fmaf(x.z, w[u + 2], acc);
                acc = fmaf(x.w, w[u + 3], acc);
            }
            part[q * d + n] = acc;
        }
    }
    __syncthreads();
    if (tid < 256) {
        float s = e.bee[tid];
#pragma unroll
        for (int q = 0; q < 4; ++q) s += part[q * d + tid];
        e1[tid] = s;
    }
    __syncthreads();
    if (tid < 64) {
        float x[4], s = 0.f;
#pragma unroll
        for (int i = 0; i < 4; ++i) { x[i] = e1[lane + 64 * i]; s += x[i]; }
#pragma unroll
        for (int o = 32; o > 0; o >>= 1) s += __shfl_xor(s, o);
        const float mean = s * (1.0f / d);
        float v = 0.f;
#pragma unroll
        for (int i = 0; i < 4; ++i) { const float t = x[i] - mean; v += t * t; }
#pragma unroll
        for (int o = 32; o > 0; o >>= 1) v += __shfl_xor(v, o);
        const float rstd = 1.0f / sqrtf(v * (1.0f / d) + 1e-5f);
#pragma unroll
        for (int i = 0; i < 4; ++i) {
            const int c = lane + 64 * i;
            e1[c] = (x[i] - mean) * rstd * e.lg[c] + e.lb[c];
        }
    }
    __syncthreads();
    {
        const int m = tid & 127, h = tid >> 7;
#pragma unroll 1
        for (int q = 2 * h; q < 2 * h + 2; ++q) {
            const float* wp = e.we2 + (size_t)32 * q * DH + m;
            float w[32];
#pragma unroll
            for (int u = 0; u < 32; ++u) w[u] = wp[u * DH];
            float acc = 0.f;
#pragma unroll
            for (int u = 0; u < 32; u += 4) {
                const float4 x = *reinterpret_cast<const float4*>(e1 + 32 * q + u);
                acc = fmaf(x.x, w[u], acc);
                acc = fmaf(x.y, w[u + 1], acc);
                acc = fmaf(x.z, w[u + 2], acc);
                acc = fmaf(x.w, w[u + 3], acc);
            }
            part[q * DH + m] = acc;
        }
    }
    __syncthreads();
    if (tid < 64) {
        float s = 0.f;
#pragma unroll
        for (int i = 0; i < 2; ++i) {
            const int mm = lane + 64 * i;
            float hsum = e.be2[mm];
#pragma unroll
            for (int q = 0; q < 8; ++q) hsum += part[q * DH + mm];
            s += fmaxf(hsum, 0.f) * e.w2[mm];
        }
#pragma unroll
        for (int o = 32; o > 0; o >>= 1) s += __shfl_xor(s, o);
        if (lane == 0) e.zemo[b] = s + e.b2[0];
    }
    __syncthreads();
}

struct EmoShape { int d = 0, DH = 0; };

__device__ __forceinline__ void emotion_layer_f4(const float* __restrict__ w, int K, int N, const float* x, float* part) {
    const int tid = threadIdx.x;
    const int tpr = N >> 2;
    const int G = 512 / tpr;
    const int c4 = tid & (tpr - 1), g = tid / tpr;
    const int kc = (K + G - 1) / G;
    const int k0 = g * kc, k1 = (k0 + kc) < K ? (k0 + kc) : K;
    float4 acc = make_float4(0.f, 0.f, 0.f, 0.f);
    const float* wp = w + 4 * c4;
    for (int k = k0; k < k1; k += 16) {
        float4 wv[16];
#pragma unroll
        for (int u = 0; u < 16; ++u) wv[u] = (k + u) < k1 ? *reinterpret_cast<const float4*>(wp + (size_t)(k + u) * N) : make_float4(0.f, 0.f, 0.f, 0.f);
#pragma unroll
        for (int u = 0; u < 16; ++u) {
            const float xv = (k + u) < k1 ? x[k + u] : 0.f;
            acc.x = fmaf(xv, wv[u].x, acc.x); acc.y = fmaf(xv, wv[u].y, acc.y);
            acc.z = fmaf(xv, wv[u].z, acc.z); acc.w = fmaf(xv, wv[u].w, acc.w);
        }
    }
    *reinterpret_cast<float4*>(part + g * N + 4 * c4) = acc;
}

__device__ __forceinline__ void emotion_window_generic(const EmoArgs& e, const EmoShape sh, int64_t b, float* scratch) {
    const int d = sh.d, DH = sh.DH;
    float* emo_s = scratch;
    float* e1 = scratch + 256;
    float* part = e1 + d;
    const int tid = threadIdx.x, lane = tid & 63;
    if (tid < 256) emo_s[tid] = tid < e.ED ? e.emo[b * e.ED + tid] : 0.f;
    __syncthreads();
    emotion_layer_f4(e.wee_t, e.ED, d, emo_s, part);
    __syncthreads();
    {
        const int G1 = 2048 / d;
        for (int n = tid; n < d; n += 512) {
            float s = e.bee[n];
            for (int g = 0; g < G1; ++g) s += part[g * d + n];
            e1[n] = s;
        }
    }
    __syncthreads();
    if (tid < 64) {
        float s = 0.f;
        for (int n = lane; n < d; n += 64) s += e1[n];
#pragma unroll
        for (int o = 32; o > 0; o >>= 1) s += __shfl_xor(s, o);
        const float mean = s / d;
        float v = 0.f;
        for (int n = lane; n < d; n += 64) { const float t = e1[n] - mean; v += t * t; }
#pragma unroll
        for (int o = 32; o > 0; o >>= 1) v += __shfl_xor(v, o);
        const float rstd = 1.0f / sqrtf(v / d + 1e-5f);
        for (int n = lane; n < d; n += 64) e1[n] = (e1[n] - mean) * rstd * e.lg[n] + e.lb[n];
    }
    __syncthreads();
    emotion_layer_f4(e.we2, d, DH, e1, part);
    __syncthreads();
    if (tid < 64) {
        const int G2 = 2048 / DH;
        float s = 0.f;
        for (int m = lane; m < DH; m += 64) {
            float h = e.be2[m];
            for (int g = 0; g < G2; ++g) h += part[g * DH + m];
            s += fmaxf(h, 0.f) * e.w2[m];
        }
#pragma unroll
        for (int o = 32; o > 0; o >>= 1) s += __shfl_xor(s, o);
        if (lane == 0) e.zemo[b] = s + e.b2[0];
    }
    __syncthreads();
}

}
```

koemorph_amd/csrc/km_host.cpp:

```cpp
#include <cctype>
#include <cmath>
#include <cstdlib>
#include <cstdarg>
#include <cstdio>
#include <cstring>

#include "km_context.h"
#include "km_kmmf.h"

namespace km {

const int kMouthIdx[kNumMouth] = {14, 15, 16, 17, 18, 19, 20, 21, 22, 23, 24, 25, 26, 27,
                                  28, 29, 30, 31, 32, 33, 34, 35, 36, 37, 38, 39, 40, 51};
const int kExprIdx[kNumExpr] = {0, 1, 2, 3, 4, 5, 6, 7, 8, 9, 10, 11, 12, 13,
                                41, 42, 43, 44, 45, 46, 47, 48, 49, 50};

static thread_local char g_err[512] = "";

void set_error(const char* fmt, ...) {
    va_list ap;
    va_start(ap, fmt);
    vsnprintf(g_err, sizeof(g_err), fmt, ap);
    va_end(ap);
}
// ... 486 lines not shown
            const double fk = (double)k * cfg.sample_rate / N;
            const double lower = (fk - mel_f[i]) / fd0, upper = (mel_f[i + 2] - fk) / fd1;
            const double v = std::fmax(0.0, std::fmin(lower, upper));
            const float v32 = (float)v;
            const float wv = (float)((double)v32 * enorm);
            row[k] = wv;
            if (wv != 0.0f) { if (first < 0) first = k; last = k; }
        }
        p->fb_offset[i] = (int32_t)p->fb_weight.size();
        if (first >= 0) {
            p->fb_start[i] = first;
            p->fb_count[i] = last - first + 1;
            for (int k = first; k <= last; ++k) p->fb_weight.push_back(row[k]);
        }
    }
    if (p->fb_weight.empty()) p->fb_weight.push_back(0.0f);
    {
        const int ng = (nm + 3) / 4;
        std::vector<int> gsteps(ng, 0), order(ng);
        auto fsteps = [&](int i) { return (i < nm && p->fb_count[i] > 0) ? ((p->fb_start[i] & 3) + p->fb_count[i] + 3) / 4 : 0; };
        for (int g = 0; g < ng; ++g) {
            for (int s = 0; s < 4; ++s) gsteps[g] = std::max(gsteps[g], fsteps(4 * g + s));
            order[g] = g;
        }
        std::stable_sort(order.begin(), order.end(), [&](int x, int y) { return gsteps[x] > gsteps[y]; });
        std::vector<std::vector<int>> mine(kMelRpWaves);
        std::vector<int> load(kMelRpWaves, 0);
        const bool fits = ng <= kMelRpWaves * kMelRpGroups;
        for (int oi = 0; fits && oi < ng; ++oi) {
            int best = -1;
            for (int w = 0; w < kMelRpWaves; ++w)
                if ((int)mine[w].size() < kMelRpGroups && (best < 0 || load[w] < load[best])) best = w;
            mine[best].push_back(order[oi]);
            load[best] += gsteps[order[oi]];
        }
        if (fits) {
            p->fbg_gid.assign((size_t)kMelRpWaves * kMelRpGroups, -1);
            p->fbg_desc.assign((size_t)kMelRpWaves * kMelRpGroups * 4, 0);
            for (int w = 0; w < kMelRpWaves; ++w)
                for (size_t gi = 0; gi < mine[w].size(); ++gi) {
                    const int g = mine[w][gi], steps = gsteps[g];
                    p->fbg_gid[(size_t)w * kMelRpGroups + gi] = g;
                    for (int s = 0; s < 4; ++s) {
                        const int i = 4 * g + s;
                        const bool live = i < nm && p->fb_count[i] > 0;
                        const int st4 = live ? (p->fb_start[i] & ~3) : 0, lead = live ? p->fb_start[i] - st4 : 0;
                        const size_t off = p->fbg_weight.size();
                        p->fbg_weight.resize(off + (size_t)4 * steps, 0.0f);
                        for (int k = 0; live && k < p->fb_count[i]; ++k) p->fbg_weight[off + lead + k] = 0.25f * p->fb_weight[p->fb_offset[i] + k];
                        p->fbg_desc[((size_t)w * kMelRpGroups + gi) * 4 + s] =
                            (int32_t)((uint32_t)(st4 / 4) | ((uint32_t)steps << 8) | ((uint32_t)(off / 4) << 16));
                        p->fbg_extent = std::max(p->fbg_extent, st4 + 4 * steps);
                    }
                }
            if (p->fbg_extent > kMelRpRow || p->fbg_weight.size() / 4 > 65535) { p->fbg_gid.clear(); p->fbg_desc.clear(); }
        }
        if (p->fbg_weight.empty()) p->fbg_weight.assign(4, 0.0f);
    }
    return p;
}

static bool same_cfg(const km_mel_config& a, const km_mel_config& b) { return std::memcmp(&a, &b, sizeof(a)) == 0; }

MelPlan* find_or_add_plan(Context* c, const km_mel_config& cfg) {
    for (MelPlan* p : c->mel_plans)
        if (same_cfg(p->cfg, cfg)) return p;
    MelPlan* p = build_mel_plan(cfg);
    c->mel_plans.push_back(p);
    return p;
}

}

using namespace km;

namespace km { const char* last_error(); }

namespace km {
namespace {
struct OptName { const char* name; int Options::*field; };
const OptName kOptNames[] = {
    {"core_split", &Options::core_split}, {"seq_per_window", &Options::seq_per_window},
    {"generic_staged", &Options::generic_staged}, {"mel_two_frame", &Options::mel_two_frame},
    {"emotion_separate", &Options::emotion_separate}, {"no_ln_fusion", &Options::no_ln_fusion},
    {"no_db_fusion", &Options::no_db_fusion}, {"no_score_fusion", &Options::no_score_fusion},
    {"no_out_fusion", &Options::no_out_fusion}, {"no_v_fusion", &Options::no_v_fusion}, {"no_core_merge", &Options::no_core_merge}, {"legacy_no_merge", &Options::legacy_no_merge}, {"kmm_no_fuse", &Options::kmm_no_fuse}, {"legacy_no_attn_fusion", &Options::legacy_no_attn_fusion}, {"legacy_no_enc_fusion", &Options::legacy_no_enc_fusion}, {"legacy_no_tail_fusion", &Options::legacy_no_tail_fusion},
    {"train_no_split", &Options::train_no_split}, {"train_tail_groups", &Options::train_tail_groups}, {"train_bm32_below", &Options::train_bm32_below}, {"train_op_per_launch", &Options::train_op_per_launch}, {"train_split_min_k", &Options::train_split_min_k}, {"train_no_dma", &Options::train_no_dma}, {"train_attn_regs", &Options::train_attn_regs}, {"train_no_fe_pack", &Options::train_no_fe_pack}, {"train_colsum_gemm", &Options::train_colsum_gemm}, {"train_no_ln_fuse", &Options::train_no_ln_fuse}, {"train_ln_fuse_rows", &Options::train_ln_fuse_rows}, {"train_no_dy_split", &Options::train_no_dy_split}, {"train_alone_max", &Options::train_alone_max},
};
}

void options_from_env(Options& o) {
    for (const OptName& n : kOptNames) {
        std::string env = "KM_";
        for (const char* p = n.name; *p; ++p) env += (char)std::toupper((unsigned char)*p);
        if (const char* v = std::getenv(env.c_str())) o.*(n.field) = *v ? std::atoi(v) : 1;
    }
    if (std::getenv("KM_GENERIC_NO_LN_FUSION")) o.no_ln_fusion = 1;
    if (std::getenv("KM_GENERIC_NO_DB_FUSION")) o.no_db_fusion = 1;
    if (std::getenv("KM_GENERIC_NO_SCORE_FUSION")) o.no_score_fusion = 1;
    if (std::getenv("KM_GENERIC_NO_OUT_FUSION")) o.no_out_fusion = 1;
    if (std::getenv("KM_GENERIC_NO_V_FUSION")) o.no_v_fusion = 1;
}

int set_option(Context* c, const char* name, long long value) {
    for (const OptName& n : kOptNames)
        if (std::strcmp(n.name, name) == 0) {
            c->opt.*(n.field) = (int)value;
            return KM_OK;
        }
    return fail(KM_ERR_INVALID_ARG, "km_set_option: unknown option '%s'", name);
}
}

extern "C" {

int km_abi_version(void) { return KM_ABI_VERSION; }
const char* km_last_error(void) { return km::last_error(); }

static void expect(Context* c, const char* key, std::vector<int64_t> shape) {
    HostParam hp;
    hp.shape = std::move(shape);
    size_t n = 1;
    for (int64_t s : hp.shape) n *= (size_t)s;
    hp.data.assign(n, 0.0f);
    c->params[key] = std::move(hp);
    c->param_order.push_back(key);
}

static int check_mel_cfg(const km_mel_config& m) {
    if (m.n_fft != 512 && m.n_fft != 1024) return fail(KM_ERR_UNSUPPORTED, "n_fft must be 512 or 1024 (got %d)", m.n_fft);
    if (m.hop_length <= 0) return fail(KM_ERR_INVALID_ARG, "invalid hop_length %d", m.hop_length);
    if (m.n_mels <= 0 || m.n_mels > 128) return fail(KM_ERR_UNSUPPORTED, "n_mels must be in 1..128 (got %d)", m.n_mels);
    if (!(m.f_max > m.f_min) || m.f_min < 0 || m.f_max > m.sample_rate / 2.0f + 1e-3f)
        return fail(KM_ERR_INVALID_ARG, "need 0 <= f_min < f_max <= sr/2");
    return KM_OK;
}


int km_set_option(km_handle h, const char* name, int64_t value) {
    if (!h || !name) return km::fail(KM_ERR_INVALID_ARG, "km_set_option: NULL argument");
    return km::set_option(h, name, (long long)value);
}

int km_create(const km_config* cfg, km_handle* out) {
    if (!cfg || !out) return fail(KM_ERR_INVALID_ARG, "km_create: NULL argument");
    if (cfg->abi_version != KM_ABI_VERSION) return fail(KM_ERR_INVALID_ARG, "km_config.abi_version %d != %d", cfg->abi_version, KM_ABI_VERSION);
    if (cfg->d_model <= 0 || cfg->num_heads <= 0 || cfg->d_model % cfg->num_heads != 0)
        return fail(KM_ERR_INVALID_ARG, "embed_dim %d must be divisible by num_heads %d", cfg->d_model, cfg->num_heads);
    if (cfg->d_model % 2 != 0 || cfg->mel_sequence_length <= 0 || cfg->emotion_dim <= 0)
        return fail(KM_ERR_INVALID_ARG, "bad d_model / mel_sequence_length / emotion_dim");
    if (cfg->num_blendshapes != 52 || cfg->num_mel_channels <= 0 || cfg->mel_temporal_frames != 3)
        return fail(KM_ERR_UNSUPPORTED, "num_blendshapes must be 52 and mel_temporal_frames 3 (ARKit grouping, dual_stream_attention.py:14-45)");
    if (cfg->num_mel_channels != cfg->mel.n_mels) return fail(KM_ERR_INVALID_ARG, "num_mel_channels != mel.n_mels");
    if (int rc = check_mel_cfg(cfg->mel)) return rc;
    km_context* c = new km_context();
    options_from_env(c->opt);
    c->cfg = *cfg;
    c->d = cfg->d_model; c->H = cfg->num_heads; c->hd = c->d / c->H; c->T = cfg->mel_sequence_length;
    c->KT = c->T + cfg->mel_temporal_frames; c->ED = cfg->emotion_dim; c->DH = c->d / 2;
    c->NB = cfg->num_blendshapes; c->NK = cfg->num_mel_channels;
    const int64_t d = c->d;
    expect(c, "mouth_queries", {kNumMouth, d});
    expect(c, "expression_queries", {kNumExpr, d});
    expect(c, "mel_weights", {c->NB});
    expect(c, "emotion_weights", {c->NB});
    expect(c, "mel_channel_encoder.weight", {d, c->KT});
    expect(c, "mel_channel_encoder.bias", {d});
// ... 216 lines not shown
```

koemorph_amd/csrc/km_mel.hip:

```cpp
#include <hip/hip_runtime.h>

#include <cstdlib>

#include "km_context.h"
#include "km_device.h"

namespace km {

#define HIP_TRY(expr)                                                                         \
    do {                                                                                      \
        hipError_t e_ = (expr);                                                               \
        if (e_ != hipSuccess) {                                                                                                        \
            (void)hipGetLastError();  \
            return fail(KM_ERR_HIP, "%s: %s", #expr, hipGetErrorString(e_));                                                           \
        }                                                                                                                              \
    } while (0)

namespace mel {
constexpr int FPB = 16;
constexpr int WAVES = 4;
constexpr int FFT_BUF = 1152;
}

__device__ __forceinline__ float2 cadd(float2 a, float2 b) { return make_float2(a.x + b.x, a.y + b.y); }
// ... 955 lines not shown
    if (p->uploaded) return KM_OK;
    if (int rc = upload(&p->d_window, p->window)) return rc;
    if (int rc = upload(&p->d_twiddle, p->twiddle)) return rc;
    if (int rc = upload(&p->d_fb_start, p->fb_start)) return rc;
    if (int rc = upload(&p->d_fb_count, p->fb_count)) return rc;
    if (int rc = upload(&p->d_fb_offset, p->fb_offset)) return rc;
    if (int rc = upload(&p->d_fb_weight, p->fb_weight)) return rc;
    if (!p->fbg_gid.empty()) {
        if (int rc = upload(&p->d_fbg_gid, p->fbg_gid)) return rc;
        if (int rc = upload(&p->d_fbg_desc, p->fbg_desc)) return rc;
        if (int rc = upload(&p->d_fbg_weight, p->fbg_weight)) return rc;
    }
    p->uploaded = true;
    return KM_OK;
}

void free_mel_plan(MelPlan* p) {
    if (p->uploaded) {
        (void)hipFree(p->d_window); (void)hipFree(p->d_twiddle); (void)hipFree(p->d_fb_start);
        (void)hipFree(p->d_fb_count); (void)hipFree(p->d_fb_offset); (void)hipFree(p->d_fb_weight);
        (void)hipFree(p->d_fbg_gid); (void)hipFree(p->d_fbg_desc); (void)hipFree(p->d_fbg_weight);
    }
    delete p;
}

static size_t melrp_lds_bytes(int nnz4) {
    return (size_t)(melrp::WAVES * melrp::FFT_BUF * 2 + melrp::FPB * melrp::NFS + melrp::WAVES + 4 + nnz4) * sizeof(float);
}

static size_t mel_lds_bytes(int nfft, int n_mels = 128, int nnz = 0) {
    if (nnz == 0) nnz = 2 * (nfft / 2 + 1) + 4 * 128;
    return (size_t)(mel::WAVES * mel::FFT_BUF * 2 + mel::FPB * (nfft / 2 + 2) + mel::FPB * n_mels + mel::WAVES +
                    3 * n_mels + nnz) * sizeof(float);
}

static LogParams log_params(const km_mel_config& m) {
    LogParams lp;
    lp.log_mode = m.log_mode; lp.amin = m.amin; lp.top_db = m.top_db; lp.db_add = m.db_add;
    lp.db_scale = m.db_scale; lp.log_eps = m.log_eps;
    return lp;
}

int growth_refused(void* stream, const char* what, int64_t need, int64_t cap) {
    hipStreamCaptureStatus cs = hipStreamCaptureStatusNone;
    if (hipStreamIsCapturing((hipStream_t)stream, &cs) == hipSuccess && cs != hipStreamCaptureStatusNone)
        return fail(KM_ERR_WORKSPACE, "%s: %lld exceeds the %lld allocated during a stream capture: run one call with this span first",
                    what, (long long)need, (long long)cap);
    return KM_OK;
}

int grow_buffer(void* ptr_addr, int64_t* cap, int64_t need, size_t unit_bytes, void* stream, const char* what) {
    void** ptr = static_cast<void**>(ptr_addr);
    if (need <= *cap) return KM_OK;
    if (int rc = growth_refused(stream, what, need, *cap)) return rc;
    if (*ptr) { HIP_TRY(hipStreamSynchronize((hipStream_t)stream)); HIP_TRY(hipFree(*ptr)); *ptr = nullptr; *cap = 0; }
    HIP_TRY(hipMalloc(ptr, (size_t)need * unit_bytes));
    *cap = need;
    return KM_OK;
}

int ensure_chunk_counters(Context* c, int64_t windows, void* stream) {
    if (windows <= c->ws_chunkctr_cap) return KM_OK;
    const int64_t cap_n = windows < 4096 ? 4096 : windows;
    if (int rc = grow_buffer(&c->ws_chunkctr, &c->ws_chunkctr_cap, cap_n, sizeof(unsigned), stream, "front end: windows of one launch")) return rc;
    HIP_TRY(hipMemsetAsync(c->ws_chunkctr, 0, (size_t)cap_n * sizeof(unsigned), (hipStream_t)stream));
    HIP_TRY(hipStreamSynchronize((hipStream_t)stream));
    return KM_OK;
}

bool mel_rp_ok(Context* c, MelPlan* p) { return p->cfg.n_fft == 1024 && !c->opt.mel_two_frame && p->d_fbg_gid != nullptr; }

bool clip_frames_shared(Context* c, MelPlan* p) {
    const km_mel_config& m = p->cfg;
    return m.pad_mode == KM_PAD_CONSTANT && 2 * m.hop_length >= m.n_fft && m.n_mels == c->NK && c->NK % 4 == 0;
}

bool mel_fuses_emotion(Context* c, MelPlan* p) {
    auto pow2 = [](int v) { return v >= 64 && v <= 1024 && (v & (v - 1)) == 0; };
    static const bool generic_ok = std::getenv("KM_EMOTION_GENERIC_SEPARATE") == nullptr;
    const bool d256 = c->d == 256 && c->DH == 128;
    return mel_rp_ok(c, p) && !c->opt.emotion_separate && c->kind == 0 && c->ED <= 256 && (d256 || (generic_ok && pow2(c->d) && pow2(c->DH)));
}

bool mel_packs(Context* c, MelPlan* p, int64_t n_frames, int64_t T) {
    const km_mel_config& m = p->cfg;
    return mel_rp_ok(c, p) && m.log_mode == KM_LOG_DB_MAX && m.top_db == m.db_add && m.db_scale > 0.f && n_frames >= T && n_frames >= 3;
}

static void mel_plan_args(MelPlan* p, MelArgs& a) {
    const km_mel_config& m = p->cfg;
    a.hop = m.hop_length; a.pad_mode = m.pad_mode;
    a.n_mels = m.n_mels; a.window = p->d_window; a.twiddle = reinterpret_cast<const float2*>(p->d_twiddle);
    a.fb_start = p->d_fb_start; a.fb_count = p->d_fb_count; a.fb_offset = p->d_fb_offset; a.fb_weight = p->d_fb_weight;
    a.fb_nnz = (int)p->fb_weight.size();
    a.fbg_gid = p->d_fbg_gid; a.fbg_desc = p->d_fbg_desc; a.fbg_weight = p->d_fbg_weight; a.fbg_nw = (int)p->fbg_weight.size();
}

int launch_mel_power(Context* c, MelPlan* p, const MelSrc& src, void* stream, const MelCarry& carry) {
    const km_mel_config& m = p->cfg;
    const SeqFrames* seq = carry.seq;
    const int64_t B = src.B, L = src.L;
    const int64_t n_frames = seq ? seq->n_rows : 1 + L / m.hop_length;
    if (m.pad_mode == KM_PAD_REFLECT && L <= m.n_fft / 2)
        return fail(KM_ERR_INVALID_ARG, "reflect padding needs more than n_fft/2 = %d samples (got %lld)", m.n_fft / 2, (long long)L);
    if (!seq && (B > c->ws_windows || n_frames > c->ws_frames))
        return fail(KM_ERR_WORKSPACE, "workspace holds %lld windows x %lld frames, need %lld x %lld: call km_reserve",
                    (long long)c->ws_windows, (long long)c->ws_frames, (long long)B, (long long)n_frames);
    if (!seq && m.n_mels > c->ws_mels)
        return fail(KM_ERR_WORKSPACE, "workspace rows hold %d mel bins, this plan has %d: call km_reserve", c->ws_mels, m.n_mels);
    const bool ring = src.ring_start != nullptr, plain = !ring && src.wins_per_clip <= 1;
    if ((carry.emotion != nullptr) + (seq != nullptr) + (carry.pack != nullptr) > 1 || (seq && !(mel_rp_ok(c, p) && !ring)) ||
        (carry.pack && !(plain && mel_packs(c, p, n_frames, carry.pack->T) && carry.pack->KP >= carry.pack->T + 3)) ||
        (carry.emotion && !(mel_fuses_emotion(c, p) && carry.zemo && src.wins_per_clip <= 1)))
        return fail(KM_ERR_UNSUPPORTED, "launch_mel_power: emotion rider, frame image or packed output requested for an unsupported configuration");
    if (!p->uploaded) return fail(KM_ERR_NOT_FINALIZED, "mel plan not uploaded (km_finalize / km_reserve first)");
    static PerDeviceOnce once;
    if (once.first(c->device)) {
        const struct { const void* fn; int lds; } kernels[] = {
            {(const void*)&mel_power_kernel<1024, false>, (int)mel_lds_bytes(1024)}, {(const void*)&mel_power_kernel<512, false>, (int)mel_lds_bytes(512)},
            {(const void*)&mel_power_kernel<1024, true>, (int)mel_lds_bytes(1024)}, {(const void*)&mel_power_kernel<512, true>, (int)mel_lds_bytes(512)},
            {(const void*)&mel_power_rp_kernel<false>, 160 * 1024}, {(const void*)&mel_power_rp_kernel<true>, 160 * 1024},
            {(const void*)&mel_power_rp_kernel<false, true>, 160 * 1024}};
        for (const auto& k : kernels) HIP_TRY(hipFuncSetAttribute(k.fn, hipFuncAttributeMaxDynamicSharedMemorySize, k.lds));
    }
    hipStream_t st = (hipStream_t)stream;
    if (int rc = ensure_chunk_counters(c, B, stream)) return rc;
    if (!seq && c->melmax_dirty) {
        HIP_TRY(hipMemsetAsync(c->ws_melmax, 0, (size_t)c->ws_windows * sizeof(unsigned), st));
        c->melmax_dirty = false;
    }
    MelArgs a;
    mel_plan_args(p, a);
    a.audio = src.audio; a.L = L; a.clip_len = src.clip_len; a.win_step = src.win_step; a.win0 = src.win0;
    a.wins_per_clip = src.wins_per_clip > 0 ? src.wins_per_clip : 1; a.n_frames = (int)n_frames;
    a.ring_start = src.ring_start; a.ready = src.ready;
    a.melpow = c->ws_melpow; a.melmax = c->ws_melmax;
    a.frame_mul = 1; a.frame_max = nullptr; a.chunk_ctr = c->ws_chunkctr;
    a.pack_xt = nullptr; a.pack_T = a.pack_KP = 0; a.pack_amin = m.amin;
    a.tab_start = nullptr; a.tab_edge = nullptr; a.tab_min = a.tab_T = a.tab_span_wgs = 0;
    if (carry.pack) { a.pack_xt = carry.pack->xt; a.pack_T = carry.pack->T; a.pack_KP = carry.pack->KP; }
    if (seq) { a.melpow = seq->pow; a.frame_max = seq->fmax; a.frame_mul = seq->frame_mul; a.melmax = nullptr; }
    if (carry.emotion) {
        auto dvp = [&](const char* name) { return (const float*)c->packed.at(name).dev; };
        a.emo.emo = carry.emotion; a.emo.ED = c->ED; a.emo.zemo = carry.zemo;
        a.emo.d = c->d; a.emo.DH = c->DH;
        a.emo.wee_t = (c->d == 256 && c->DH == 128) ? dvp("wee_t256") : dvp("wee_t"); a.emo.bee = dvp("bee"); a.emo.lg = dvp("eln_g"); a.emo.lb = dvp("eln_b");
        a.emo.we2 = dvp("we2"); a.emo.be2 = dvp("be2"); a.emo.w2 = dvp("w2"); a.emo.b2 = dvp("b2");
    }
    const int n_chunks = (int)((n_frames + mel::FPB - 1) / mel::FPB);
    int per_window = (int)((512 + B / 2) / B);
    if (per_window > n_chunks) per_window = n_chunks;
    if (per_window < 1) per_window = 1;
    const dim3 grid((unsigned)per_window, (unsigned)B);
    if (mel_rp_ok(c, p)) {
        const size_t ldsrp = melrp_lds_bytes(a.fbg_nw);
        if (carry.pack) hipLaunchKernelGGL((mel_power_rp_kernel<false, true>), grid, dim3(melrp::NT), ldsrp, st, a);
        else if (!ring) hipLaunchKernelGGL((mel_power_rp_kernel<false>), grid, dim3(melrp::NT), ldsrp, st, a);
        else hipLaunchKernelGGL((mel_power_rp_kernel<true>), grid, dim3(melrp::NT), ldsrp, st, a);
        HIP_TRY(hipGetLastError());
        return KM_OK;
    }
    const size_t lds = mel_lds_bytes(m.n_fft, m.n_mels, a.fb_nnz);
    if (m.n_fft == 1024 && !ring) hipLaunchKernelGGL((mel_power_kernel<1024, false>), grid, dim3(256), lds, st, a);
    else if (m.n_fft == 1024) hipLaunchKernelGGL((mel_power_kernel<1024, true>), grid, dim3(256), lds, st, a);
    else if (!ring) hipLaunchKernelGGL((mel_power_kernel<512, false>), grid, dim3(256), lds, st, a);
    else hipLaunchKernelGGL((mel_power_kernel<512, true>), grid, dim3(256), lds, st, a);
    HIP_TRY(hipGetLastError());
    return KM_OK;
}

struct ClipPackArgs {
    const float* span;
    int edge_off;
    const int* start;
    int min_start, n_span, T, KP, n_mels, row_stride, tile_cols;
    float amin;
    float* xt;
    unsigned* melmax;
};
namespace clippack {
constexpr int NT = 1024, MAXI = 24, LDS_FLOATS = 24 * 1024;
inline int row_stride(int n_mels) { return (n_mels + 45) / 64 * 64 + 18; }
inline int tile_cols(int n_mels, int KP) {
    int c = NT * MAXI / n_mels;
    const int l = LDS_FLOATS / row_stride(n_mels);
    c = (c < l ? c : l) / 32 * 32;
    return c < KP ? c : KP;
}
}

__global__ __launch_bounds__(clippack::NT) void train_clip_pack_kernel(ClipPackArgs a) {
    using namespace clippack;
    extern __shared__ __attribute__((aligned(16))) float smem[];
    __shared__ float redmax[NT / 64];
    const int tid = threadIdx.x, b = blockIdx.x;
    int s = a.start[b];
    s = s < 0 ? 0 : s;
    const int row0 = s - a.min_start;
    const int e0 = a.edge_off + b * 2 * a.n_mels;
    const int dq = NT / a.n_mels, dr = NT % a.n_mels;
    const int cl0 = tid / a.n_mels, m0 = tid - cl0 * a.n_mels;
    float vmax = 0.f;
    for (int c0 = 0; c0 < a.KP; c0 += a.tile_cols) {
        const int ncol = a.KP - c0 < a.tile_cols ? a.KP - c0 : a.tile_cols;
        const int total = ncol * a.n_mels;
        float pwv[MAXI];
        int cl = cl0, m = m0;
#pragma unroll
        for (int k = 0; k < MAXI; ++k) {
            const int col = c0 + cl;
            const int f = col < a.T ? col : col - 2;
            pwv[k] = -1.f;
            if (tid + k * NT < total && col < a.T + 3) {
                int r = row0 + f;
                r = r < 0 ? 0 : (r >= a.n_span ? a.n_span - 1 : r);
                pwv[k] = a.span[(f == 0 ? e0 : (f == a.T ? e0 + a.n_mels : r * a.n_mels)) + m];
            }
            cl += dq; m += dr;
            if (m >= a.n_mels) { m -= a.n_mels; ++cl; }
        }
        if (c0 > 0) __syncthreads();
        cl = cl0; m = m0;
#pragma unroll
        for (int k = 0; k < MAXI; ++k) {
            if (tid + k * NT < total) {
                const float pw = pwv[k];
                vmax = fmaxf(vmax, pw);
                smem[cl * a.row_stride + m] = pw >= 0.f ? db10(pw, a.amin) : 0.f;
            }
            cl += dq; m += dr;
            if (m >= a.n_mels) { m -= a.n_mels; ++cl; }
// ... 140 lines not shown
```

koemorph_amd/streaming.py:

```python
from __future__ import annotations

import ctypes as C
from typing import Optional, Tuple

import torch

from . import _lib
from ._lib import check
from .engine import Engine, MelConfig, _ptr, _stream_ptr


def stream_shape(context_window: float, update_interval: float, mel_hop: int, sample_rate: int = 16000) -> dict:
    ring_len = int(context_window * sample_rate)
    return dict(ring_len=ring_len, ring_hop=int(sample_rate / (1.0 / update_interval)), n_frames=1 + ring_len // mel_hop,
                stream_out_frames=int(context_window / update_interval))


class StreamEngine:
    def __init__(self, engine: Engine, n_streams: int, context_window: float = 8.5, update_interval: float = 0.0333,
                 mel: Optional[MelConfig] = None):
        if engine.device is None:
            raise _lib.KoeMorphError(_lib.KM_ERR_NOT_FINALIZED, "finalize the Engine before creating streams")
        self.engine = engine
        self.n_streams = n_streams
        self.mel = mel or MelConfig.sliding_window(n_fft=1024, hop_length=engine.mel.hop_length)
        self._lib = engine._lib
        cfg = self.mel.to_c()
        with torch.cuda.device(engine.device):
            check(self._lib.km_stream_create(engine._h, n_streams, context_window, update_interval, C.byref(cfg)))
        self.shape = stream_shape(context_window, update_interval, self.mel.hop_length, self.mel.sample_rate)
        self.ring_hop = self.shape["ring_hop"]
        dev = engine.device
        self.out = torch.zeros(n_streams, engine.num_blendshapes, device=dev)
        self.ready = torch.zeros(n_streams, dtype=torch.uint8, device=dev)
        self._graph = None
        self._g_samples = self._g_emotion = None

    def push(self, samples: torch.Tensor) -> None:
        if samples.dim() != 2 or samples.shape[0] != self.n_streams:
            raise ValueError(f"expected ({self.n_streams}, n) samples, got {tuple(samples.shape)}")
        samples = samples.contiguous()
        check(self._lib.km_stream_push(self.engine._h, _ptr(samples), samples.shape[1], _stream_ptr(samples.device)))

    def tick(self, emotion: torch.Tensor) -> Tuple[torch.Tensor, torch.Tensor]:
        emotion = emotion.contiguous()
        check(self._lib.km_stream_tick(self.engine._h, _ptr(emotion), _ptr(self.out), _ptr(self.ready),
                                       _stream_ptr(emotion.device)))
        return self.out, self.ready

    def reset(self) -> None:
        check(self._lib.km_stream_reset(self.engine._h, _stream_ptr(self.engine.device)))
        self.out.zero_()
        self.ready.zero_()

    def capture(self, n_per_stream: Optional[int] = None, host_out: Optional[torch.Tensor] = None) -> None:
        dev = self.engine.device
        if n_per_stream is None:
            n_per_stream = 533 if abs(533 - self.ring_hop) <= 1 else self.ring_hop + 1
        if host_out is not None and (not host_out.is_pinned() or tuple(host_out.shape) != tuple(self.out.shape)):
            raise ValueError("host_out must be a pinned host tensor of the shape of the result")
        self._g_samples = torch.zeros(self.n_streams, n_per_stream, device=dev)
        self._g_emotion = torch.zeros(self.n_streams, self.engine.emotion_dim, device=dev)
        torch.cuda.synchronize(dev)
        g = torch.cuda.CUDAGraph()
        with torch.cuda.graph(g):
            self.push(self._g_samples)
            self.tick(self._g_emotion)
            if host_out is not None:
                host_out.copy_(self.out, non_blocking=True)
        self._graph = g
        self._g_host_out = host_out

    def replay(self, samples: torch.Tensor, emotion: torch.Tensor) -> Tuple[torch.Tensor, torch.Tensor]:
        if self._graph is None:
            raise RuntimeError("capture() first")
        self._g_samples.copy_(samples, non_blocking=True)
        self._g_emotion.copy_(emotion, non_blocking=True)
        self._graph.replay()
        return self.out, self.ready


def legacy_stream_shape(buffer_duration: float = 2.0, audio_length: int = 16000, hop: int = 533, sample_rate: int = 16000) -> dict:
    buffer_samples = int(buffer_duration * sample_rate)
    if audio_length <= 0 or buffer_samples <= 0 or hop <= 0:
        raise ValueError("buffer_duration, audio_length and hop must be positive")
    if audio_length > buffer_samples:
        raise ValueError(f"audio_length {audio_length} exceeds the buffer of {buffer_samples} samples: no read could ever succeed")
    n_frames = 1 + audio_length // hop
    return dict(buffer_samples=buffer_samples, n_frames=n_frames, supported=n_frames <= 32)


class LegacyStreamEngine:

    def __init__(self, model, n_streams: int, buffer_duration: float = 2.0, audio_length: int = 16000):
        lib, h, dev = model._handle()
        self.model, self.n_streams, self.audio_length = model, n_streams, audio_length
        self._lib, self._h, self.device = lib, h, dev
        self.shape = legacy_stream_shape(buffer_duration, audio_length, model.hop_length, model.sample_rate)
        self.buffer_samples = self.shape["buffer_samples"]
        with torch.cuda.device(dev):
            torch.cuda.synchronize(dev)
            check(lib.km_legacy_stream_create(h, n_streams, self.buffer_samples, audio_length))
        model._reserved = (max(model._reserved[0], n_streams), max(model._reserved[1], audio_length))
        self.out = torch.zeros(n_streams, model.num_blendshapes, device=dev)
        self.ready = torch.zeros(n_streams, dtype=torch.uint8, device=dev)
        self._graph = None
        self._g_samples = self._g_counts = self._g_host_out = None

    def push(self, samples: torch.Tensor, counts: Optional[torch.Tensor] = None) -> None:
        if samples.dim() != 2 or samples.shape[0] != self.n_streams or samples.dtype != torch.float32:
            raise ValueError(f"expected ({self.n_streams}, n) float32 samples, got {tuple(samples.shape)} {samples.dtype}")
        if counts is not None and (counts.dtype != torch.int32 or tuple(counts.shape) != (self.n_streams,)):
            raise ValueError(f"expected ({self.n_streams},) int32 counts")
        samples = samples.contiguous()
        check(self._lib.km_legacy_stream_push(self._h, _ptr(samples), samples.shape[1],
                                              _ptr(counts.contiguous()) if counts is not None else None, _stream_ptr(samples.device)))

    def tick(self) -> Tuple[torch.Tensor, torch.Tensor]:
        check(self._lib.km_legacy_stream_tick(self._h, _ptr(self.out), _ptr(self.ready), _stream_ptr(self.device)))
        return self.out, self.ready

    def reset(self) -> None:
        check(self._lib.km_legacy_stream_reset(self._h, _stream_ptr(self.device)))
        self.out.zero_()
        self.ready.zero_()

    def capture(self, n_per_stream: int, host_out: Optional[torch.Tensor] = None) -> None:
        dev = self.device
        if host_out is not None and (not host_out.is_pinned() or tuple(host_out.shape) != tuple(self.out.shape)):
            raise ValueError("host_out must be a pinned host tensor of the shape of the result")
        self._g_samples = torch.zeros(self.n_streams, n_per_stream, device=dev)
        self._g_counts = torch.full((self.n_streams,), n_per_stream, dtype=torch.int32, device=dev)
        torch.cuda.synchronize(dev)
        g = torch.cuda.CUDAGraph()
        with torch.cuda.graph(g):
            self.push(self._g_samples, self._g_counts)
# ... 20 lines not shown
```

Before: 1.870 million frames/s.

## Compute emotion logit inside fused core kernel, interleaved with mel/attention phases

```diff
diff --git a/include/koemorph.h b/include/koemorph.h
--- a/include/koemorph.h
+++ b/include/koemorph.h
@@ -227,6 +227,7 @@
 int km_stream_push(km_handle h, const float* samples_dev, int64_t n_per_stream, void* stream);
 int km_stream_tick(km_handle h, const float* emotion_dev, float* out_dev, uint8_t* ready_dev, void* stream);
 int km_stream_reset(km_handle h, void* stream);
+int km_stream_reset_one(km_handle h, int64_t index, void* stream);
 
 int km_legacy_stream_create(km_handle h, int64_t n_streams, int64_t buffer_samples, int64_t audio_length);
 int km_legacy_stream_push(km_handle h, const float* samples_dev, int64_t n_per_stream, const int32_t* counts_dev, void* stream);
diff --git a/koemorph_amd/_lib.py b/koemorph_amd/_lib.py
--- a/koemorph_amd/_lib.py
+++ b/koemorph_amd/_lib.py
@@ -153,6 +153,7 @@
     "km_stream_push": (C.c_int, [_h, _p, _i64, _p]),
     "km_stream_tick": (C.c_int, [_h, _p, _p, _p, _p]),
     "km_stream_reset": (C.c_int, [_h, _p]),
+    "km_stream_reset_one": (C.c_int, [_h, _i64, _p]),
     "km_legacy_stream_create": (C.c_int, [_h, _i64, _i64, _i64]),
     "km_legacy_stream_push": (C.c_int, [_h, _p, _i64, _p, _p]),
     "km_legacy_stream_tick": (C.c_int, [_h, _p, _p, _p]),
diff --git a/koemorph_amd/csrc/km_api.hip b/koemorph_amd/csrc/km_api.hip
--- a/koemorph_amd/csrc/km_api.hip
+++ b/koemorph_amd/csrc/km_api.hip
@@ -808,14 +808,16 @@
     }
     hipStream_t st = (hipStream_t)stream;
     const bool tm = c->stage_timing;
-    const bool fuse_emo = mel_fuses_emotion(c, plan);
+    const bool core_emo = core_computes_emotion(c, plan);
+    const bool fuse_emo = !core_emo && mel_fuses_emotion(c, plan);
     if (tm) HIP_TRY(hipEventRecord((hipEvent_t)c->stage_ev[0], st));
-    if (!fuse_emo)
+    if (!core_emo && !fuse_emo)
         if (int rc = launch_emotion(c, emotion_dev, B, c->ws_zemo, stream)) return rc;
     if (tm) HIP_TRY(hipEventRecord((hipEvent_t)c->stage_ev[1], st));
     if (int rc = launch_mel_power(c, plan, src, stream, fuse_emo ? mel_emotion(emotion_dev, c->ws_zemo) : MelCarry{})) return rc;
     if (tm) { HIP_TRY(hipEventRecord((hipEvent_t)c->stage_ev[2], st)); HIP_TRY(hipEventRecord((hipEvent_t)c->stage_ev[3], st)); }
-    if (int rc = launch_core_fused_db(c, plan, B, n_frames, c->ws_zemo, out_dev, stream, core_workspace(state_dev, first))) return rc;
+    if (int rc = launch_core_fused_db(c, plan, B, n_frames, c->ws_zemo, out_dev, stream,
+                                      core_with_emotion(core_workspace(state_dev, first), core_emo ? emotion_dev : nullptr))) return rc;
     if (tm) HIP_TRY(hipEventRecord((hipEvent_t)c->stage_ev[4], st));
     return KM_OK;
 }
@@ -883,6 +885,21 @@
     return KM_OK;
 }
 
+int km_stream_reset_one(km_handle h, int64_t index, void* stream) {
+    if (int rc = need_dual(h)) return rc;
+    Context* c = h;
+    if (c->n_streams <= 0) return fail(KM_ERR_INVALID_ARG, "km_stream_reset_one: no streams (km_stream_create first)");
+    if (index < 0 || index >= c->n_streams) return fail(KM_ERR_INVALID_ARG, "km_stream_reset_one: stream %lld of %lld", (long long)index, (long long)c->n_streams);
+    hipStream_t st = (hipStream_t)stream;
+    HIP_TRY(hipMemsetAsync(c->ring + index * c->ring_len, 0, (size_t)c->ring_len * sizeof(float), st));
+    HIP_TRY(hipMemsetAsync(c->ring_wptr + index, 0, sizeof(int), st));
+    HIP_TRY(hipMemsetAsync(c->ring_frames + index, 0, sizeof(int), st));
+    HIP_TRY(hipMemsetAsync(c->ring_ready + index, 0, 1, st));
+    HIP_TRY(hipMemsetAsync(c->ring_started + index, 0, 1, st));
+    HIP_TRY(hipMemsetAsync(c->ring_state + index * c->NB, 0, (size_t)c->NB * sizeof(float), st));
+    return KM_OK;
+}
+
 int km_stream_create(km_handle h, int64_t n_streams, double context_window_s, double update_interval_s,
                      const km_mel_config* mel_cfg) {
     if (int rc = need_dual(h)) return rc;
@@ -934,12 +951,14 @@
     const int64_t S = c->n_streams, L = c->ring_len;
     const int64_t n_frames = 1 + L / c->stream_plan->cfg.hop_length;
     if (S > c->ws_windows || n_frames > c->ws_frames) return fail(KM_ERR_WORKSPACE, "stream workspace too small");
-    const bool fuse_emo = mel_fuses_emotion(c, c->stream_plan);
-    if (!fuse_emo)
+    const bool core_emo = core_computes_emotion(c, c->stream_plan);
+    const bool fuse_emo = !core_emo && mel_fuses_emotion(c, c->stream_plan);
+    if (!core_emo && !fuse_emo)
         if (int rc = launch_emotion(c, emotion_dev, S, c->ws_zemo, stream)) return rc;
     if (int rc = launch_mel_power(c, c->stream_plan, mel_rings(c), stream, fuse_emo ? mel_emotion(emotion_dev, c->ws_zemo) : MelCarry{})) return rc;
     if (c->fused_ok) {
-        if (int rc = launch_core_fused_db(c, c->stream_plan, S, n_frames, c->ws_zemo, out_dev, stream, core_stream(c))) return rc;
+        if (int rc = launch_core_fused_db(c, c->stream_plan, S, n_frames, c->ws_zemo, out_dev, stream,
+                                          core_with_emotion(core_stream(c), core_emo ? emotion_dev : nullptr))) return rc;
     } else {
         if (int rc = launch_core512_stream(c, c->stream_plan, S, n_frames, c->ws_zemo, out_dev, stream)) return rc;
     }
@@ -1118,15 +1137,17 @@
         if (hipEventRecord((hipEvent_t)c->pipe_ev_in[slot], caller) != hipSuccess) { rc = fail(KM_ERR_HIP, "hipEventRecord failed"); break; }
         if (hipStreamWaitEvent(s1, (hipEvent_t)c->pipe_ev_in[slot], 0) != hipSuccess) { rc = fail(KM_ERR_HIP, "hipStreamWaitEvent failed"); break; }
         if (tm) (void)hipEventRecord((hipEvent_t)c->stage_ev[0], s1);
-        const bool fuse_emo = mel_fuses_emotion(c, c->mel_plans[0]);
-        if (!fuse_emo && (rc = launch_emotion(c, emotion_dev, B, c->ws_zemo, s1))) break;
+        const bool core_emo = core_computes_emotion(c, c->mel_plans[0]);
+        const bool fuse_emo = !core_emo && mel_fuses_emotion(c, c->mel_plans[0]);
+        if (!core_emo && !fuse_emo && (rc = launch_emotion(c, emotion_dev, B, c->ws_zemo, s1))) break;
         if (tm) (void)hipEventRecord((hipEvent_t)c->stage_ev[1], s1);
         if ((rc = launch_mel_power(c, c->mel_plans[0], mel_windows(audio_dev, B, L), s1, fuse_emo ? mel_emotion(emotion_dev, c->ws_zemo) : MelCarry{}))) break;
         if (tm) (void)hipEventRecord((hipEvent_t)c->stage_ev[2], s1);
         (void)hipEventRecord((hipEvent_t)c->pipe_ev_mel[slot], s1);
         (void)hipStreamWaitEvent(s2, (hipEvent_t)c->pipe_ev_mel[slot], 0);
         if (tm) (void)hipEventRecord((hipEvent_t)c->stage_ev[3], s2);
-        if ((rc = launch_core_fused_db(c, c->mel_plans[0], B, n_frames, c->ws_zemo, out_dev, s2, core_workspace(state_dev, first)))) break;
+        if ((rc = launch_core_fused_db(c, c->mel_plans[0], B, n_frames, c->ws_zemo, out_dev, s2,
+                                       core_with_emotion(core_workspace(state_dev, first), core_emo ? emotion_dev : nullptr)))) break;
         if (tm) (void)hipEventRecord((hipEvent_t)c->stage_ev[4], s2);
         (void)hipEventRecord((hipEvent_t)c->pipe_ev_core[slot], s2);
         if (c->pipe_seq > 0) (void)hipStreamWaitEvent(caller, (hipEvent_t)c->pipe_ev_core[slot ^ 1], 0);
diff --git a/koemorph_amd/csrc/km_context.h b/koemorph_amd/csrc/km_context.h
--- a/koemorph_amd/csrc/km_context.h
+++ b/koemorph_amd/csrc/km_context.h
@@ -60,6 +60,7 @@
     int generic_staged = 0;
     int mel_two_frame = 0;
     int emotion_separate = 0;
+    int emotion_in_front_end = 0;
     int no_ln_fusion = 0, no_db_fusion = 0, no_score_fusion = 0, no_out_fusion = 0, no_v_fusion = 0;
     int legacy_no_merge = 0;
     int no_core_merge = 0;
@@ -215,12 +216,15 @@
     const unsigned char* ready; unsigned char* started;
     const SeqCore* seq;
     const ClipTable* tab;
+    const float* emotion;
 };
 inline CoreSrc core_workspace(float* state, int first) { return {state, first, 0, 1, 0, nullptr, nullptr, nullptr, nullptr}; }
 inline CoreSrc core_workspace_seq(int64_t win0, int n_per_clip) { return {nullptr, 1, win0, n_per_clip, 0, nullptr, nullptr, nullptr, nullptr}; }
 inline CoreSrc core_strided(const SeqCore* s, int64_t win0) { return {nullptr, 1, win0, s->n_per_clip, 0, nullptr, nullptr, s, nullptr}; }
 inline CoreSrc core_table(const ClipTable* t, float* state, int first) { return {state, first, 0, 1, 0, nullptr, nullptr, nullptr, t}; }
 inline CoreSrc core_stream(Context* c) { return {c->ring_state, 0, 0, 1, c->stream_out_frames, c->ring_ready, c->ring_started, nullptr, nullptr}; }
+inline CoreSrc core_with_emotion(CoreSrc s, const float* emotion) { s.emotion = emotion; return s; }
+bool core_computes_emotion(Context* c, MelPlan* p);
 int launch_core_fused_db(Context* c, MelPlan* p, int64_t B, int64_t n_frames, const float* zemo, float* out, void* stream,
                          const CoreSrc& src);
 int launch_seq_window_max(Context* c, const unsigned* fmax, const unsigned* emax, int64_t nw, int64_t win0, int nfc, int stride,
@@ -308,6 +312,8 @@
 int launch_train_clip_pack(Context* c, MelPlan* p, const float* span, const float* edge, const int* start_frames, int64_t B,
                            int min_start, int64_t n_span, int T, int KP, float* xt, void* stream);
 bool mel_fuses_emotion(Context* c, MelPlan* p);
+struct EmoArgs;
+void emotion_rider_args(Context* c, const float* emotion, float* zemo, EmoArgs& e);
 int ensure_chunk_counters(Context* c, int64_t windows, void* stream);
 int growth_refused(void* stream, const char* what, int64_t need, int64_t cap);
 int grow_buffer(void* ptr_addr, int64_t* cap, int64_t need, size_t unit_bytes, void* stream, const char* what);
diff --git a/koemorph_amd/csrc/km_core.hip b/koemorph_amd/csrc/km_core.hip
--- a/koemorph_amd/csrc/km_core.hip
+++ b/koemorph_amd/csrc/km_core.hip
@@ -26,13 +26,14 @@
 constexpr int KB = 16;
 constexpr int R1_FLOATS = KTP * NK;
 constexpr int R2_FLOATS = 2 * NW * NK + 2 * NK;
-constexpr int LDS_BYTES = (R1_FLOATS + R2_FLOATS) * 4;
+constexpr int R3_FLOATS = 1536;
+constexpr int LDS_BYTES = (R1_FLOATS + R2_FLOATS + R3_FLOATS) * 4;
 constexpr int YSB = 264;
 constexpr int PLANE_FLOATS = NK * YSB / 2;
 constexpr int XSB = 296, XKB = 9;
 constexpr int XPLANE_FLOATS = NK * XSB / 2;
 constexpr int r1_floats(int np) { return np * XPLANE_FLOATS > R1_FLOATS ? np * XPLANE_FLOATS : R1_FLOATS; }
-constexpr int lds_bytes(int np) { return (r1_floats(np) + R2_FLOATS) * 4; }
+constexpr int lds_bytes(int np) { return (r1_floats(np) + R2_FLOATS + R3_FLOATS) * 4; }
 }
 
 typedef __bf16 bf16x8 __attribute__((ext_vector_type(8)));
@@ -66,6 +67,7 @@
     unsigned char* started;
     const int* seq_start;
     int seq_min;
+    EmoArgs emo;
 };
 
 __device__ __forceinline__ int mouth_slot_of(int i) { return (i >= 14 && i <= 40) ? i - 14 : (i == 51 ? 27 : -1); }
@@ -76,6 +78,7 @@
     extern __shared__ __attribute__((aligned(16))) float smem[];
     float* R1 = smem;
     float* R2 = smem + r1_floats(NP);
+    float* R3 = R2 + R2_FLOATS;
 
     const int b = blockIdx.x;
     const int tid = threadIdx.x;
@@ -98,6 +101,10 @@
 #pragma unroll
     for (int r = 0; r < 4; ++r) { bf4[r] = a.bf[16 * wave + 4 * g + r]; w24[r] = a.w2[16 * wave + 4 * g + r]; }
     const float tail_b2 = a.b2[0], tail_ws = tid < 52 ? a.wsum[tid] : 0.f;
+
+    const EmoStream256 es(a.emo, R3);
+    float z_emo = 0.f;
+    bool own_logit = false;
 
     if constexpr (FUSE_DB) {
         float ref_db, floor_db;
@@ -124,7 +131,9 @@
         };
         float4* dst = reinterpret_cast<float4*>(R1);
         const float4 z4 = make_float4(0.f, 0.f, 0.f, 0.f);
+        own_logit = a.emo.emo != nullptr;
         if constexpr (NP > 0) {
+            if (own_logit) z_emo = emotion_logit_d256(a.emo, a.win0 + b, R3);
             auto src_row = [&](int t) -> int {
                 if (t < T) return t < tv ? (t < F ? t : F - 1) : -1;
                 if (t >= T + 3) return -1;
@@ -174,23 +183,37 @@
         constexpr int NLD = T * 20 / NT;
         static_assert(NLD * NT == T * 20, "phase 0 assumes T*20 is a multiple of the workgroup size");
         float4 xv[NLD];
-#pragma unroll
-        for (int u = 0; u < NLD; ++u) {
-            const int i = tid + NT * u;
-            int fr = i / 20;
-            const int c4 = i - fr * 20;
-            fr = fr < F ? fr : F - 1;
-            xv[u] = i < tv * 20 ? row4(fr)[c4] : z4;
-        }
         float4 sv = z4;
         bool s_ok = false;
-        if (tid < 60) {
-            const int r = tid / 20;
-            int fr = -1;
-            if (U >= 3) fr = U - 3 + r; else if (r < U) fr = r;
-            if (fr >= F) fr = F - 1;
-            s_ok = fr >= 0;
-            if (s_ok) sv = row4(fr)[tid - r * 20];
+        auto request_rows = [&]() {
+#pragma unroll
+            for (int u = 0; u < NLD; ++u) {
+                const int i = tid + NT * u;
+                int fr = i / 20;
+                const int c4 = i - fr * 20;
+                fr = fr < F ? fr : F - 1;
+                xv[u] = i < tv * 20 ? row4(fr)[c4] : z4;
+            }
+            if (tid < 60) {
+                const int r = tid / 20;
+                int fr = -1;
+                if (U >= 3) fr = U - 3 + r; else if (r < U) fr = r;
+                if (fr >= F) fr = F - 1;
+                s_ok = fr >= 0;
+                if (s_ok) sv = row4(fr)[tid - r * 20];
+            }
+        };
+        float ew[64];
+        if (own_logit) {
+            const float ev = es.load_row(a.win0 + b);
+            es.request_l1(2 * es.h1(), ew);
+            request_rows();
+            es.stage_row(ev);
+            __syncthreads();
+            es.l1_quarter(2 * es.h1(), ew);
+            es.request_l1(2 * es.h1() + 1, ew);
+        } else {
+            request_rows();
         }
         auto convert = [&](auto mode) {
             constexpr int MODE = decltype(mode)::value;
@@ -204,6 +227,7 @@
         if (a.lp.log_mode == KM_LOG_LN_EPS) convert(std::integral_constant<int, KM_LOG_LN_EPS>{});
         else convert(std::integral_constant<int, KM_LOG_DB_MAX>{});
         if (tid >= 64 && tid < 64 + (KTP - KT) * 20) dst[KT * 20 + tid - 64] = z4;
+        if (own_logit) es.l1_quarter(2 * es.h1() + 1, ew);
         }
     } else {
         const int tv = a.t_in < T ? a.t_in : T;
@@ -219,6 +243,9 @@
     __syncthreads();
     if constexpr (FUSE_DB) {
         if (tid == 0) a.melmax[b] = 0u;
+        if constexpr (NP == 0) {
+            if (own_logit) es.sum_l1();
+        }
     }
 
     f32x4 acc[5][2];
@@ -291,6 +318,10 @@
         const f32x4* vp0 = reinterpret_cast<const f32x4*>(a.wv_p) + (size_t)wave * KB * 2 * 64 + lane;
         q0 = qp0[0]; q1 = qp0[64]; v0 = vp0[0]; v1 = vp0[64];
     }
+    float ew2[2][32];
+    if constexpr (FUSE_DB && NP == 0) {
+        if (own_logit) { es.request_l2(2 * es.h2(), ew2[0]); es.request_l2(2 * es.h2() + 1, ew2[1]); }
+    }
     {
 #pragma unroll
         for (int mt = 0; mt < 5; ++mt)
@@ -322,6 +353,12 @@
                 for (int r = 0; r < 4; ++r) P[(16 * mt + 4 * g + r) * NW + wave] = part[mt][r];
         }
         __syncthreads();
+        if constexpr (FUSE_DB && NP == 0) {
+            if (own_logit) {
+                if (pass == 0) es.layer_norm();
+                else z_emo = es.finish();
+            }
+        }
         float* Tt = R2 + 2 * NW * NK + pass * NK;
         if (lane < NK / NW) {
             const int row = wave * (NK / NW) + lane;
@@ -333,6 +370,9 @@
             Tt[row] = s;
         }
         __syncthreads();
+        if constexpr (FUSE_DB && NP == 0) {
+            if (pass == 0 && own_logit) { es.l2_eighth(2 * es.h2(), ew2[0]); es.l2_eighth(2 * es.h2() + 1, ew2[1]); }
+        }
 #pragma unroll
         for (int mt = 0; mt < 5; ++mt) {
             const f32x4 t4 = *reinterpret_cast<const f32x4*>(Tt + 16 * mt + 4 * g);
@@ -553,7 +593,7 @@
 #pragma unroll
             for (int w = 0; w < NW; ++w) z += R2[w * 32 + slot];
         } else {
-            z = a.zemo[(a.win0 + b) / a.zemo_div];
+            z = (FUSE_DB && a.emo.emo) ? z_emo : a.zemo[(a.win0 + b) / a.zemo_div];
         }
         const float bs = 1.0f / (1.0f + expf(-z));
         float val = fminf(fmaxf(tail_ws * bs, 0.f), 1.f);
@@ -930,6 +970,10 @@
     return KM_OK;
 }
 
+bool core_computes_emotion(Context* c, MelPlan* p) {
+    return c->fused_ok && c->d == 256 && c->DH == 128 && !c->opt.emotion_in_front_end && mel_fuses_emotion(c, p);
+}
+
 int launch_core_fused_db(Context* c, MelPlan* p, int64_t B, int64_t n_frames, const float* zemo, float* out, void* stream,
                          const CoreSrc& src) {
     if (int rc = core_attrs(c)) return rc;
@@ -939,6 +983,11 @@
     a.out = out; a.state = src.state; a.first = src.first; a.win0 = src.win0; a.zemo_div = src.zemo_div > 0 ? src.zemo_div : 1;
     a.melpow = c->ws_melpow; a.melmax = c->ws_melmax; a.n_frames = (int)n_frames; a.lp = plan_log_params(p);
     a.n_use = (int)(src.n_use > 0 ? src.n_use : n_frames); a.ready = src.ready; a.started = src.started;
+    if (src.emotion) {
+        if (!core_computes_emotion(c, p) || src.seq || src.tab || a.zemo_div != 1)
+            return fail(KM_ERR_UNSUPPORTED, "fused core: emotion features given to a launch that reads its logits (sequence, table or switched off)");
+        emotion_rider_args(c, src.emotion, nullptr, a.emo);
+    }
     if (const SeqCore* s = src.seq) { a.seq_pow = s->pow; a.seq_edge = s->edge; a.seq_nfc = s->nfc; a.seq_stride = s->stride; a.seq_n = s->n_per_clip; }
     if (const ClipTable* t = src.tab) {
         if (src.seq || c->opt.core_split == 3 || c->opt.core_split == 6)
diff --git a/koemorph_amd/csrc/km_device.h b/koemorph_amd/csrc/km_device.h
--- a/koemorph_amd/csrc/km_device.h
+++ b/koemorph_amd/csrc/km_device.h
@@ -90,98 +90,131 @@
     int d = 256, DH = 128;
 };
 
+struct EmoStream256 {
+    static constexpr int d = 256, DH = 128;
+    const EmoArgs& e;
+    float *emo_s , *e1 , *part ;
+    __device__ __forceinline__ EmoStream256(const EmoArgs& e_, float* scratch) : e(e_), emo_s(scratch), e1(scratch + 256), part(scratch + 512) {}
+    __device__ __forceinline__ int h1() const { return __builtin_amdgcn_readfirstlane((int)threadIdx.x >> 8); }
+    __device__ __forceinline__ int h2() const { return (int)threadIdx.x >> 7; }
+    __device__ __forceinline__ float load_row(int64_t b) const { const int tid = threadIdx.x; return tid < e.ED ? e.emo[b * e.ED + tid] : 0.f; }
+    __device__ __forceinline__ void stage_row(float v) const { if (threadIdx.x < 256) emo_s[threadIdx.x] = v; }
+    __device__ __forceinline__ void request_l1(int q, float (&w)[64]) const {
+        const float* wp = e.wee_t + (size_t)64 * q * d + (threadIdx.x & 255);
+#pragma unroll
+        for (int u = 0; u < 64; ++u) w[u] = wp[u * d];
+    }
+    __device__ __forceinline__ void l1_quarter(int q, const float (&w)[64]) const {
+        float acc = 0.f;
+#pragma unroll
+        for (int u = 0; u < 64; u += 4) {
+            const float4 x = *reinterpret_cast<const float4*>(emo_s + 64 * q + u);
+            acc = fmaf(x.x, w[u], acc);
+            acc = fmaf(x.y, w[u + 1], acc);
+            acc = fmaf(x.z, w[u + 2], acc);
+            acc = fmaf(x.w, w[u + 3], acc);
+        }
+        part[q * d + (threadIdx.x & 255)] = acc;
+    }
+    __device__ __forceinline__ void sum_l1() const {
+        const int tid = threadIdx.x;
+        if (tid < 256) {
+            float s = e.bee[tid];
+#pragma unroll
+            for (int q = 0; q < 4; ++q) s += part[q * d + tid];
+            e1[tid] = s;
+        }
+    }
+    __device__ __forceinline__ void layer_norm() const {
+        const int tid = threadIdx.x, lane = tid & 63;
+        if (tid < 64) {
+            float x[4], s = 0.f;
+#pragma unroll
+            for (int i = 0; i < 4; ++i) { x[i] = e1[lane + 64 * i]; s += x[i]; }
+#pragma unroll
+            for (int o = 32; o > 0; o >>= 1) s += __shfl_xor(s, o);
+            const float mean = s * (1.0f / d);
+            float v = 0.f;
+#pragma unroll
+            for (int i = 0; i < 4; ++i) { const float t = x[i] - mean; v = fmaf(t, t, v); }
+#pragma unroll
+            for (int o = 32; o > 0; o >>= 1) v += __shfl_xor(v, o);
+            const float rstd = 1.0f / sqrtf(v * (1.0f / d) + 1e-5f);
+#pragma unroll
+            for (int i = 0; i < 4; ++i) {
+                const int c = lane + 64 * i;
+                e1[c] = fmaf((x[i] - mean) * rstd, e.lg[c], e.lb[c]);
+            }
+        }
+    }
+    __device__ __forceinline__ void request_l2(int q, float (&w)[32]) const {
+        const float* wp = e.we2 + (size_t)32 * q * DH + (threadIdx.x & 127);
+#pragma unroll
+        for (int u = 0; u < 32; ++u) w[u] = wp[u * DH];
+    }
+    __device__ __forceinline__ void l2_eighth(int q, const float (&w)[32]) const {
+        float acc = 0.f;
+#pragma unroll
+        for (int u = 0; u < 32; u += 4) {
+            const float4 x = *reinterpret_cast<const float4*>(e1 + 32 * q + u);
+            acc = fmaf(x.x, w[u], acc);
+            acc = fmaf(x.y, w[u + 1], acc);
+            acc = fmaf(x.z, w[u + 2], acc);
+            acc = fmaf(x.w, w[u + 3], acc);
+        }
+        part[q * DH + (threadIdx.x & 127)] = acc;
+    }
+    __device__ __forceinline__ float finish() const {
+        const int tid = threadIdx.x, lane = tid & 63;
+        float z = 0.f;
+        if (tid < 64) {
+            float s = 0.f;
+#pragma unroll
+            for (int i = 0; i < 2; ++i) {
+                const int mm = lane + 64 * i;
+                float hsum = e.be2[mm];
+#pragma unroll
+                for (int q = 0; q < 8; ++q) hsum += part[q * DH + mm];
+                s = fmaf(fmaxf(hsum, 0.f), e.w2[mm], s);
+            }
+#pragma unroll
+            for (int o = 32; o > 0; o >>= 1) s += __shfl_xor(s, o);
+            z = s + e.b2[0];
+        }
+        return z;
+    }
+};
+
+__device__ __forceinline__ float emotion_logit_d256(const EmoArgs& e, int64_t b, float* scratch) {
+    const EmoStream256 es(e, scratch);
+    es.stage_row(es.load_row(b));
+    __syncthreads();
+#pragma unroll 1
+    for (int q = 2 * es.h1(); q < 2 * es.h1() + 2; ++q) {
+        float w[64];
+        es.request_l1(q, w);
+        es.l1_quarter(q, w);
+    }
+    __syncthreads();
+    es.sum_l1();
+    __syncthreads();
+    es.layer_norm();
+    __syncthreads();
+#pragma unroll 1
+    for (int q = 2 * es.h2(); q < 2 * es.h2() + 2; ++q) {
+        float w[32];
+        es.request_l2(q, w);
+        es.l2_eighth(q, w);
+    }
+    __syncthreads();
+    const float z = es.finish();
+    __syncthreads();
+    return z;
+}
+
 __device__ __forceinline__ void emotion_window_d256(const EmoArgs& e, int64_t b, float* scratch) {
-    constexpr int d = 256, DH = 128;
-    float* emo_s = scratch;
-    float* e1 = scratch + 256;
-    float* part = scratch + 512;
-    const int tid = threadIdx.x, lane = tid & 63;
-    if (tid < 256) emo_s[tid] = tid < e.ED ? e.emo[b * e.ED + tid] : 0.f;
-    __syncthreads();
-    {
-        const int n = tid & 255, h = __builtin_amdgcn_readfirstlane(tid >> 8);
-#pragma unroll 1
-        for (int q = 2 * h; q < 2 * h + 2; ++q) {
-            const float* wp = e.wee_t + (size_t)64 * q * d + n;
-            float w[64];
-#pragma unroll
-            for (int u = 0; u < 64; ++u) w[u] = wp[u * d];
-            float acc = 0.f;
-#pragma unroll
-            for (int u = 0; u < 64; u += 4) {
-                const float4 x = *reinterpret_cast<const float4*>(emo_s + 64 * q + u);
-                acc = fmaf(x.x, w[u], acc);
-                acc = fmaf(x.y, w[u + 1], acc);
-                acc = fmaf(x.z, w[u + 2], acc);
-                acc = fmaf(x.w, w[u + 3], acc);
-            }
-            part[q * d + n] = acc;
-        }
-    }
-    __syncthreads();
-    if (tid < 256) {
-        float s = e.bee[tid];
-#pragma unroll
-        for (int q = 0; q < 4; ++q) s += part[q * d + tid];
-        e1[tid] = s;
-    }
-    __syncthreads();
-    if (tid < 64) {
-        float x[4], s = 0.f;
-#pragma unroll
-        for (int i = 0; i < 4; ++i) { x[i] = e1[lane + 64 * i]; s += x[i]; }
-#pragma unroll
-        for (int o = 32; o > 0; o >>= 1) s += __shfl_xor(s, o);
-        const float mean = s * (1.0f / d);
-        float v = 0.f;
-#pragma unroll
-        for (int i = 0; i < 4; ++i) { const float t = x[i] - mean; v += t * t; }
-#pragma unroll
-        for (int o = 32; o > 0; o >>= 1) v += __shfl_xor(v, o);
-        const float rstd = 1.0f / sqrtf(v * (1.0f / d) + 1e-5f);
-#pragma unroll
-        for (int i = 0; i < 4; ++i) {
-            const int c = lane + 64 * i;
-            e1[c] = (x[i] - mean) * rstd * e.lg[c] + e.lb[c];
-        }
-    }
-    __syncthreads();
-    {
-        const int m = tid & 127, h = tid >> 7;
-#pragma unroll 1
-        for (int q = 2 * h; q < 2 * h + 2; ++q) {
-            const float* wp = e.we2 + (size_t)32 * q * DH + m;
-            float w[32];
-#pragma unroll
-            for (int u = 0; u < 32; ++u) w[u] = wp[u * DH];
-            float acc = 0.f;
-#pragma unroll
-            for (int u = 0; u < 32; u += 4) {
-                const float4 x = *reinterpret_cast<const float4*>(e1 + 32 * q + u);
-                acc = fmaf(x.x, w[u], acc);
-                acc = fmaf(x.y, w[u + 1], acc);
-                acc = fmaf(x.z, w[u + 2], acc);
-                acc = fmaf(x.w, w[u + 3], acc);
-            }
-            part[q * DH + m] = acc;
-        }
-    }
-    __syncthreads();
-    if (tid < 64) {
-        float s = 0.f;
-#pragma unroll
-        for (int i = 0; i < 2; ++i) {
-            const int mm = lane + 64 * i;
-            float hsum = e.be2[mm];
-#pragma unroll
-            for (int q = 0; q < 8; ++q) hsum += part[q * DH + mm];
-            s += fmaxf(hsum, 0.f) * e.w2[mm];
-        }
-#pragma unroll
-        for (int o = 32; o > 0; o >>= 1) s += __shfl_xor(s, o);
-        if (lane == 0) e.zemo[b] = s + e.b2[0];
-    }
-    __syncthreads();
+    const float z = emotion_logit_d256(e, b, scratch);
+    if (threadIdx.x == 0) e.zemo[b] = z;
 }
 
 struct EmoShape { int d = 0, DH = 0; };
diff --git a/koemorph_amd/csrc/km_host.cpp b/koemorph_amd/csrc/km_host.cpp
--- a/koemorph_amd/csrc/km_host.cpp
+++ b/koemorph_amd/csrc/km_host.cpp
@@ -592,7 +592,7 @@
 const OptName kOptNames[] = {
     {"core_split", &Options::core_split}, {"seq_per_window", &Options::seq_per_window},
     {"generic_staged", &Options::generic_staged}, {"mel_two_frame", &Options::mel_two_frame},
-    {"emotion_separate", &Options::emotion_separate}, {"no_ln_fusion", &Options::no_ln_fusion},
+    {"emotion_separate", &Options::emotion_separate}, {"emotion_in_front_end", &Options::emotion_in_front_end}, {"no_ln_fusion", &Options::no_ln_fusion},
     {"no_db_fusion", &Options::no_db_fusion}, {"no_score_fusion", &Options::no_score_fusion},
     {"no_out_fusion", &Options::no_out_fusion}, {"no_v_fusion", &Options::no_v_fusion}, {"no_core_merge", &Options::no_core_merge}, {"legacy_no_merge", &Options::legacy_no_merge}, {"kmm_no_fuse", &Options::kmm_no_fuse}, {"legacy_no_attn_fusion", &Options::legacy_no_attn_fusion}, {"legacy_no_enc_fusion", &Options::legacy_no_enc_fusion}, {"legacy_no_tail_fusion", &Options::legacy_no_tail_fusion},
     {"train_no_split", &Options::train_no_split}, {"train_tail_groups", &Options::train_tail_groups}, {"train_bm32_below", &Options::train_bm32_below}, {"train_op_per_launch", &Options::train_op_per_launch}, {"train_split_min_k", &Options::train_split_min_k}, {"train_no_dma", &Options::train_no_dma}, {"train_attn_regs", &Options::train_attn_regs}, {"train_no_fe_pack", &Options::train_no_fe_pack}, {"train_colsum_gemm", &Options::train_colsum_gemm}, {"train_no_ln_fuse", &Options::train_no_ln_fuse}, {"train_ln_fuse_rows", &Options::train_ln_fuse_rows}, {"train_no_dy_split", &Options::train_no_dy_split}, {"train_alone_max", &Options::train_alone_max},
diff --git a/koemorph_amd/csrc/km_mel.hip b/koemorph_amd/csrc/km_mel.hip
--- a/koemorph_amd/csrc/km_mel.hip
+++ b/koemorph_amd/csrc/km_mel.hip
@@ -1061,6 +1061,14 @@
     return mel_rp_ok(c, p) && !c->opt.emotion_separate && c->kind == 0 && c->ED <= 256 && (d256 || (generic_ok && pow2(c->d) && pow2(c->DH)));
 }
 
+void emotion_rider_args(Context* c, const float* emotion, float* zemo, EmoArgs& e) {
+    auto dvp = [&](const char* name) { return (const float*)c->packed.at(name).dev; };
+    e.emo = emotion; e.ED = c->ED; e.zemo = zemo;
+    e.d = c->d; e.DH = c->DH;
+    e.wee_t = (c->d == 256 && c->DH == 128) ? dvp("wee_t256") : dvp("wee_t"); e.bee = dvp("bee"); e.lg = dvp("eln_g"); e.lb = dvp("eln_b");
+    e.we2 = dvp("we2"); e.be2 = dvp("be2"); e.w2 = dvp("w2"); e.b2 = dvp("b2");
+}
+
 bool mel_packs(Context* c, MelPlan* p, int64_t n_frames, int64_t T) {
     const km_mel_config& m = p->cfg;
     return mel_rp_ok(c, p) && m.log_mode == KM_LOG_DB_MAX && m.top_db == m.db_add && m.db_scale > 0.f && n_frames >= T && n_frames >= 3;
@@ -1119,13 +1127,7 @@
     a.tab_start = nullptr; a.tab_edge = nullptr; a.tab_min = a.tab_T = a.tab_span_wgs = 0;
     if (carry.pack) { a.pack_xt = carry.pack->xt; a.pack_T = carry.pack->T; a.pack_KP = carry.pack->KP; }
     if (seq) { a.melpow = seq->pow; a.frame_max = seq->fmax; a.frame_mul = seq->frame_mul; a.melmax = nullptr; }
-    if (carry.emotion) {
-        auto dvp = [&](const char* name) { return (const float*)c->packed.at(name).dev; };
-        a.emo.emo = carry.emotion; a.emo.ED = c->ED; a.emo.zemo = carry.zemo;
-        a.emo.d = c->d; a.emo.DH = c->DH;
-        a.emo.wee_t = (c->d == 256 && c->DH == 128) ? dvp("wee_t256") : dvp("wee_t"); a.emo.bee = dvp("bee"); a.emo.lg = dvp("eln_g"); a.emo.lb = dvp("eln_b");
-        a.emo.we2 = dvp("we2"); a.emo.be2 = dvp("be2"); a.emo.w2 = dvp("w2"); a.emo.b2 = dvp("b2");
-    }
+    if (carry.emotion) emotion_rider_args(c, carry.emotion, carry.zemo, a.emo);
     const int n_chunks = (int)((n_frames + mel::FPB - 1) / mel::FPB);
     int per_window = (int)((512 + B / 2) / B);
     if (per_window > n_chunks) per_window = n_chunks;
diff --git a/koemorph_amd/streaming.py b/koemorph_amd/streaming.py
--- a/koemorph_amd/streaming.py
+++ b/koemorph_amd/streaming.py
@@ -52,6 +52,9 @@
         check(self._lib.km_stream_reset(self.engine._h, _stream_ptr(self.engine.device)))
         self.out.zero_()
         self.ready.zero_()
+
+    def reset_stream(self, index: int) -> None:
+        check(self._lib.km_stream_reset_one(self.engine._h, index, _stream_ptr(self.engine.device)))
 
     def capture(self, n_per_stream: Optional[int] = None, host_out: Optional[torch.Tensor] = None) -> None:
         dev = self.engine.device
```

New measurement: 1.862 million frames/s. No clear change (-0.5%).
